# NILOIDE/A.I.gar

Measured on AMD Instinct MI355X. Metric: env-steps/sec at 4096 bots x 100k pellets; 1/2/4/8 MI355X scaling, higher is better.
Workload: dtype f64; 1 GPU; C3: 4096 bots, 100000 pellets, 1152 viruses, split p=0.0025, eject p=0.01, field 4800, obs 854 floats/bot; start: data/c3_t50.npz (tick 50, mean cell mass 17.45, max 51.3) + 30 untimed random-policy ticks to settle; policy=random, parallelism=single-gpu

## Files before the change

aigar_amd/csrc/aigar_dev.h:

```cpp
#pragma once
#include <stdint.h>

#include "../../include/aigar.h"

namespace aigar {

#ifdef AIGAR_FLOOR
#ifdef AIGAR_FLOOR_OPAQUE
#define FLOOR(k) \
  if ((((AIGAR_FLOOR) >> (k)) & 1) && d.A > 0) return
#else
#define FLOOR(k) \
  if (((AIGAR_FLOOR) >> (k)) & 1) return
#endif
#else
#define FLOOR(k)
#endif

struct ArenaCtl {
  int64_t seq_next;
  int64_t tick;
  int64_t tick_sp;
  uint64_t key0, key1, ctr_pellet, ctr_virus;
  int64_t seq_base_upd;
// ... 20 lines not shown
  double vmin_mass;
  uint64_t ev_order;
  uint32_t food_round;
  uint32_t scan_epoch[2];
  int scan_ticket[2];
  int src_n_stage;
  int n_kill;
  int pu_nconv;
  int pu_nsp, pu_spec;
  uint32_t dirty;
  int food_undone[3];
  uint32_t pl_epoch;
  int pl_ticket;
  int n_pel_glob, n_eaten_glob, n_out, n_out_pel, n_undone, n_undone_glob;
  int n_ho;
  int n_ho_live;
  int n_cmd;
  int64_t stat[8];
};

enum : uint32_t {
  ERR_PELLET_CAP = 1, ERR_BLOB_CAP = 2, ERR_VIRUS_CAP = 4, ERR_EVENT_CAP = 8, ERR_WORK_CAP = 16,
  ERR_OBS_CAP = 32, ERR_CAND_CAP = 64, ERR_SLOT = 128, ERR_PIX_CAP = 256, ERR_TILE_CAP = 512, ERR_TILE_LOOKUP = 1024,
  ERR_TILE_OBS = 2048,
  ERR_TILE_PASSES = 4096,
  ERR_PREDICT = 8192,
  ERR_TILE_HANDOFF = 16384
};
enum : uint32_t {
  WARN_NEW_VIRUS_EATS = 1, WARN_DEAD_VIRUS = 2, WARN_TILE_OBS = 4,
  WARN_Q_NONFINITE = 8,
  WARN_NOISE_NONFINITE = 16,
  WARN_NOISE_EXHAUSTED = 32,
  WARN_TRAIN_NONFINITE = 64
};
enum : uint32_t { DIRTY_VIRUS = 1, DIRTY_BLOB = 2 };

enum : uint32_t { PH_MERGE = 0, PH_VB = 1, PH_PV = 2, PH_PELLET = 3, PH_BLOB = 4, PH_PP = 5, PH_SPAWN = 6 };

struct TileRec {
  int32_t kind, idx;
  int64_t seq;
  double x, y;
};
enum : int32_t { TR_HDR = 0, TR_PELLET = 1, TR_BLOB = 2, TR_CELL = 3, TR_HIST = 4, TR_CMD = 5 };
constexpr int kHcapMax = 256;

struct alignas(32) PelRec {
  double x, y, m;
  int64_t seq;
};
constexpr int kPelStride = 4;
__device__ __forceinline__ void pel_store(PelRec *p, const PelRec &r) {
#ifdef AIGAR_PEL_WT
  __hip_atomic_store(&p->x, r.x, __ATOMIC_RELAXED, __HIP_MEMORY_SCOPE_AGENT);
  __hip_atomic_store(&p->y, r.y, __ATOMIC_RELAXED, __HIP_MEMORY_SCOPE_AGENT);
  __hip_atomic_store(&p->m, r.m, __ATOMIC_RELAXED, __HIP_MEMORY_SCOPE_AGENT);
  __hip_atomic_store(&p->seq, r.seq, __ATOMIC_RELAXED, __HIP_MEMORY_SCOPE_AGENT);
#else
  *p = r;
#endif
}

struct ScoreCtl {
  double *trace;
  int64_t cap;
};

struct Dev {
  int A, B, NP, size, cols, H;
  int tiled, tile_id, ntiles, tcap, bm_words;
  int tile_flags;
  int tile_nx, tile_ny;
  int tile_gate;
  int hcap, hrec, nh;
  int *t_holder;
  int *t_obsby;
  int *t_holive;
  uint8_t *t_hodefer;
  int *t_hoslot;
  int own_bx0, own_bx1, own_by0, own_by1;
  int loc_bx0, loc_bx1, loc_by0, loc_by1;
  TileRec *outbox;
  const TileRec *inbox;
  int *ticket;
  int *kill_list;
  double *spec_x, *spec_y, *spec_m;
  double pow_n032[17];
  int cshift;
  int cshift_c;
  int Pcap, Ecap, Vcap, Wcap, EVcap;
  int PR;
  int PS;
  int PD;
  int PH1;
  int virus_enabled;
  double max_pellets, max_viruses;
  int G, L;
  uint32_t obs_ch, obs_ex;
  int flags;
  int pp_par;
  ArenaCtl *ctl;
  int *p_alive, *p_respawn, *p_ncells, *p_split, *p_eject, *p_pend;
  double *p_cmdx, *p_cmdy;
  double *p_fx, *p_fy, *p_fs, *p_mass;
  int *p_split_lh;
  uint8_t *p_role;
  int *p_time;
  double *o_last_mass;
  uint8_t *p_list;
  int *p_newc, *p_newb, *p_seqoff, *p_bloboff;
  int *p_heavy;
  double *c_x, *c_y, *c_m, *c_r, *c_vx, *c_vy, *c_svx, *c_svy, *c_mt;
  int *c_svc;
  uint32_t *c_flags;
  int64_t *c_seq;
  uint8_t *c_active;
  double *sp_r, *sp_svx, *sp_svy;
  double *sb_x, *sb_y, *sb_svx, *sb_svy;
  uint8_t *sb_slot;
  PelRec *pel;
  int *pel_col;
  PelRec *pn;
  int *pn_col;
  uint8_t *pel_dead;
  int *pel_rank;
  int *pstart;
  int *pncnt;
  uint64_t *pel_owner;
  double *b_x, *b_y, *b_m, *b_r, *b_vx, *b_vy, *b_svx, *b_svy;
  int *b_svc;
  int64_t *b_seq, *b_ej;
  int *b_col;
  uint32_t *b_flags;
  uint64_t *b_owner;
  int *bstart, *bitems, *b_rank;
  uint64_t *bmap;
  double *v_x, *v_y, *v_m, *v_r, *v_vx, *v_vy, *v_svx, *v_svy;
  int *v_svc;
  int64_t *v_seq;
  uint32_t *v_flags;
  int *v_active;
  int *vcnt, *vstart, *vitems, *v_rank;
  int *ccnt, *cstart, *citems, *c_rank;
  int *cgcnt;
  unsigned long long *occ;
  int *occ_cnt;
  int occ_words;
  int *dead;
  int *work, *work2;
  int *f_list;
  uint8_t *f_cnt;
  uint8_t *f_done;
  int *resp_slot;
  int *resp_list;
  int64_t *ev;
  double *o_lastfov;
  double *o_self_lf, *o_self_slf, *o_en_lf, *o_en_slf;
  double *o_act_cur, *o_act_prev;
  unsigned long long *scan_state;
  unsigned long long *pl_state;
  int pl_tiles;
  int scan_tiles;
  int OBcap;
  unsigned long long *ob_used;
  uint32_t *ob_epoch;
  int64_t *ob_seq;
  double *ob_m, *ob_r;
  uint32_t *ob_mask;
  uint8_t *ob_own;
  int *ob_perm;
  uint64_t *ob_wmask;
  double *sc;
  ScoreCtl *sc_ctl;
};
enum { SC_N = 0, SC_SUM = 1, SC_MAX = 2, SC_DEAD = 3 };

struct ArenaSel {
  const int *al;
  const uint64_t *seeds;
  uint64_t seed;
  int first, n;
  __device__ __forceinline__ int arena(int i) const { return al ? al[i] : first + i; }
  __device__ __forceinline__ uint64_t seed_of(int i) const { return seeds ? seeds[i] : seed; }
  __device__ __forceinline__ int key_arena(int i) const { return al ? 0 : first + i; }
};

constexpr int FCAP = 32;

struct RandomPolicy {
  int on;
  double ps, pe;
  uint64_t salt;
};

}
```

aigar_amd/csrc/api.hip:

```cpp
#include <dlfcn.h>
#include <hip/hip_runtime.h>

#include <algorithm>
#include <cmath>
#include <cstdarg>
#include <cstdio>
#include <cstdlib>
#include <cstring>
#include <string>
#include <type_traits>
#include <vector>

#include "../../include/aigar.h"
#include "aigar_dev.h"
#include "aigar_sem.h"

namespace aigar {
void launch_tick(const Dev &d, hipStream_t s, int rounds, int64_t *scr_k, int *scr_v,
                 const RandomPolicy *rp = nullptr);
void launch_tick_pre(const Dev &d, hipStream_t s, int64_t *scr_k, int *scr_v, const RandomPolicy *rp);
void launch_tick_post(const Dev &d, hipStream_t s, int64_t *scr_k, int *scr_v);
void launch_tile_pass(const Dev &d, hipStream_t s, int rounds, int64_t *scr_k, int *scr_v, int first);
void launch_tile_policy(const Dev &d, hipStream_t s, int greedy_split, uint8_t *mask, int cap);
void launch_tile_cmd_apply(const Dev &d, hipStream_t s, int box_recs);
// ... 375 lines not shown
  if (cfg->obs_channels & AIGAR_OBS_ALL &&
      cfg->obs_channels & (AIGAR_OBS_SELF_LF | AIGAR_OBS_SELF_SLF | AIGAR_OBS_ENEMY_LF | AIGAR_OBS_ENEMY_SLF))
    return fail("aigar_create: ALL_PLAYER_GRID with last-frame grids is undefined in the reference");
  if ((cfg->flags & AIGAR_FLAG_SCORE) &&
      (std::max(1, cfg->tile_x) * std::max(1, cfg->tile_y) > 1 || (cfg->tile_flags & AIGAR_TILE_FORCE)))
    return fail("aigar_create: AIGAR_FLAG_SCORE (the mass history score) is not kept on a tiled handle");
  int ndev = 0;
  HIPCHK(hipGetDeviceCount(&ndev));
  if (cfg->device < 0 || cfg->device >= ndev) return fail("aigar_create: device %d not present (%d devices)", cfg->device, ndev);
  HIPCHK(hipSetDevice(cfg->device));
  aigar_handle *h = new aigar_handle();
  h->cfg = *cfg;
  if (getenv("AIGAR_NO_GRAPH")) h->use_graph = false;
  if (const char *u = getenv("AIGAR_RUN_UNROLL")) h->run_unroll = std::max(1, std::min(64, atoi(u)));
  if (getenv("AIGAR_TILE_GRAPH")) h->tile_graph = true;
  h->d.pp_par = getenv("AIGAR_PP_SERIAL") ? 0 : 1;
  if (const char *r = getenv("AIGAR_FOOD_ROUNDS")) h->rounds = std::max(1, std::min(16, atoi(r)));
  Dev &d = h->d;
  d.A = cfg->n_arenas;
  d.B = cfg->bots_per_arena;
  d.NP = d.A * d.B;
  d.size = cfg->field_size > 0 ? cfg->field_size : (int)(75 * std::sqrt((double)d.B));
  d.cols = (int)std::ceil(d.size / 20.0);
  d.H = d.cols * d.cols;
  d.virus_enabled = cfg->virus_enabled ? 1 : 0;
  d.max_pellets = cfg->max_pellets >= 0 ? cfg->max_pellets : (double)d.size * d.size * 0.015;
  d.max_viruses = cfg->max_viruses >= 0 ? cfg->max_viruses : (double)d.size * d.size * 0.00005;
  if (!d.virus_enabled) d.max_viruses = 0;
  auto r64 = [](int v) { return (v + 63) / 64 * 64; };
  d.Ecap = r64(cfg->blob_cap > 0 ? cfg->blob_cap : 4 * d.B + 256);
  d.Pcap = r64(cfg->pellet_cap > 0 ? cfg->pellet_cap : (int)std::ceil(d.max_pellets) + d.Ecap + 64);
  d.Vcap = r64(cfg->virus_cap > 0 ? cfg->virus_cap : 2 * (int)std::ceil(d.max_viruses) + 64);
  if (d.cols > 1024) {
    delete h;
    return fail("aigar_create: field size %d: more than 1024 bucket rows", d.size);
  }
  d.PR = r64((int)std::ceil(1.25 * d.Pcap / d.cols) + 64);
  d.PS = 2 * d.cols * d.PR;
  d.PD = d.PS + d.Pcap;
  d.PH1 = d.cols * (d.cols + 1) + 1;
  d.Wcap = std::max(kMaxCells * d.B, std::max(d.Ecap, 4096));
  d.EVcap = cfg->event_cap > 0 ? cfg->event_cap : 65536;
  d.G = G;
  d.L = obs_len_of(*cfg);
  d.obs_ch = cfg->obs_channels;
  d.obs_ex = cfg->obs_extras;
  d.flags = cfg->flags;
  d.occ_words = (d.H + 63) / 64;
  d.scan_tiles = (d.H + 2047) / 2048;
  d.pl_tiles = (d.B + 255) / 256;
  const int tx = std::max(1, cfg->tile_x), ty = std::max(1, cfg->tile_y);
  d.ntiles = tx * ty;
  d.tiled = d.ntiles > 1 || (cfg->tile_flags & AIGAR_TILE_FORCE);
  d.own_bx0 = d.own_by0 = d.loc_bx0 = d.loc_by0 = 0;
  d.own_bx1 = d.own_by1 = d.loc_bx1 = d.loc_by1 = d.cols;
  if (d.tiled) {
    auto bad = [&](const char *m) {
      delete h;
      return fail("aigar_create: %s", m);
    };
    if (d.A != 1) return bad("a tiled handle steps one arena (n_arenas must be 1)");
    if (cfg->tile_id < 0 || cfg->tile_id >= d.ntiles) return bad("tile_id out of range");
    if (tx > d.cols || ty > d.cols) return bad("more tiles than hash buckets along a side");
    const int ix = cfg->tile_id % tx, iy = cfg->tile_id / tx;
    const int halo = cfg->tile_halo > 0 ? cfg->tile_halo : 400;
    const int hb = std::max(7, (halo + kBucket - 1) / kBucket);
    if (d.ntiles > 64) return bad("at most 64 tiles");
    d.tile_id = cfg->tile_id;
    d.tile_flags = cfg->tile_flags;
    d.own_bx0 = ix * d.cols / tx;
    d.own_bx1 = (ix + 1) * d.cols / tx;
    d.own_by0 = iy * d.cols / ty;
    d.own_by1 = (iy + 1) * d.cols / ty;
    d.loc_bx0 = std::max(0, d.own_bx0 - hb);
    d.loc_bx1 = std::min(d.cols, d.own_bx1 + hb);
    d.loc_by0 = std::max(0, d.own_by0 - hb);
    d.loc_by1 = std::min(d.cols, d.own_by1 + hb);
  }
  d.tile_nx = tx;
  d.tile_ny = ty;
  d.tile_gate = 0;
  d.tcap = cfg->tile_cap > 0 ? cfg->tile_cap : 2048;
  d.bm_words = (int)(((size_t)kMaxCells * d.NP + 255) / 256 * 4);
  {
    const uint32_t ch = cfg->obs_channels;
    d.nh = ((ch & (AIGAR_OBS_SELF_LF | AIGAR_OBS_SELF_SLF)) ? 1 : 0) + ((ch & AIGAR_OBS_SELF_SLF) ? 1 : 0) +
           ((ch & (AIGAR_OBS_ENEMY_LF | AIGAR_OBS_ENEMY_SLF)) ? 1 : 0) + ((ch & AIGAR_OBS_ENEMY_SLF) ? 1 : 0);
    d.hrec = 1 + (d.nh * G * G + 3) / 4;
    d.hcap = std::min(kHcapMax, std::max(16, d.tcap / 64));
  }
  h->box_recs = 1 + d.tcap + std::max(d.bm_words / 4, d.hcap * d.hrec);
  for (int k = 0; k <= kMaxCells; k++) d.pow_n032[k] = aigar_math::pow_glibc((double)k, 0.32);
  d.cshift = 3;
  while ((((d.cols + (1 << d.cshift) - 1) >> d.cshift) * ((d.cols + (1 << d.cshift) - 1) >> d.cshift)) > 4096)
    d.cshift++;
  d.cshift_c = 0;
  while ((((d.cols + (1 << d.cshift_c) - 1) >> d.cshift_c) * ((d.cols + (1 << d.cshift_c) - 1) >> d.cshift_c)) > 4096)
    d.cshift_c++;
  if (hipStreamCreateWithFlags(&h->stream, hipStreamNonBlocking) != hipSuccess) {
    delete h;
    return fail("hipStreamCreate failed");
  }
  const size_t A = d.A, NP = d.NP, C = (size_t)kMaxCells * NP, H1 = (size_t)d.H + 1, GG = (size_t)G * G;
  bool ok = true;
#define AL(field, T, n)                     \
  do {                                      \
    d.field = dalloc<T>(h, (n));            \
    ok = ok && d.field != nullptr;          \
  } while (0)
#ifndef AIGAR_NO_ARENA
  for (int pass = 0; pass < 2; pass++) {
    h->arena_sizing = pass == 0;
    if (pass == 1) {
      h->arena_size = h->arena_used;
      h->arena_used = 0;
      void *base = nullptr;
      if (hipMalloc(&base, h->arena_size) != hipSuccess) {
        ok = false;
        break;
      }
      h->allocs.push_back(base);
      (void)hipMemset(base, 0, h->arena_size);
      h->arena = (char *)base;
    }
#endif
  AL(ctl, ArenaCtl, A);
  AL(p_alive, int, NP); AL(p_respawn, int, NP); AL(p_ncells, int, NP); AL(p_split, int, NP); AL(p_eject, int, NP);
  AL(p_pend, int, NP); AL(p_cmdx, double, NP); AL(p_cmdy, double, NP); AL(p_list, uint8_t, C);
  AL(p_newc, int, NP); AL(p_heavy, int, NP); AL(p_newb, int, NP); AL(p_seqoff, int, NP); AL(p_bloboff, int, NP);
  AL(c_x, double, C); AL(c_y, double, C); AL(c_m, double, C); AL(c_r, double, C); AL(c_vx, double, C);
  AL(c_vy, double, C); AL(c_svx, double, C); AL(c_svy, double, C); AL(c_mt, double, C); AL(c_svc, int, C);
  AL(c_flags, uint32_t, C); AL(c_seq, int64_t, C); AL(c_active, uint8_t, C);
  AL(sp_r, double, C); AL(sp_svx, double, C); AL(sp_svy, double, C);
  AL(sb_x, double, C); AL(sb_y, double, C); AL(sb_svx, double, C); AL(sb_svy, double, C); AL(sb_slot, uint8_t, C);
  const size_t P = A * d.Pcap, PSA = A * d.PS, PDA = A * d.PD, PHA = A * d.PH1;
  AL(pel, PelRec, PSA); AL(pel_col, int, PSA);
  AL(pn, PelRec, P); AL(pn_col, int, P);
  AL(pel_dead, uint8_t, PDA); AL(pel_rank, int, P); AL(pncnt, int, PHA); AL(pstart, int, PHA);
  AL(pel_owner, uint64_t, PDA);
  const size_t E = A * d.Ecap, V = A * d.Vcap;
  AL(b_x, double, E); AL(b_y, double, E); AL(b_m, double, E); AL(b_r, double, E); AL(b_vx, double, E);
  AL(b_vy, double, E); AL(b_svx, double, E); AL(b_svy, double, E); AL(b_svc, int, E); AL(b_seq, int64_t, E);
  AL(b_ej, int64_t, E); AL(b_flags, uint32_t, E); AL(b_owner, uint64_t, E); AL(b_col, int, E);
  AL(bstart, int, A * H1); AL(bitems, int, E); AL(b_rank, int, E); AL(bmap, uint64_t, A * 64);
  AL(v_x, double, V); AL(v_y, double, V); AL(v_m, double, V); AL(v_r, double, V); AL(v_vx, double, V);
  AL(v_vy, double, V); AL(v_svx, double, V); AL(v_svy, double, V); AL(v_svc, int, V); AL(v_seq, int64_t, V);
  AL(v_flags, uint32_t, V); AL(v_active, int, V);
  AL(vcnt, int, A * H1); AL(vstart, int, A * H1); AL(vitems, int, V); AL(v_rank, int, V);
  AL(ccnt, int, A * H1); AL(cstart, int, A * H1); AL(citems, int, C); AL(c_rank, int, C);
  AL(cgcnt, int, A * 2 * 4100);
  AL(occ, unsigned long long, A * d.occ_words); AL(occ_cnt, int, A * d.H);
  AL(dead, int, NP); AL(work, int, A * d.Wcap); AL(work2, int, A * d.Wcap);
  AL(f_list, int, C * FCAP); AL(f_cnt, uint8_t, C); AL(f_done, uint8_t, C);
  AL(resp_slot, int, NP); AL(resp_list, int, NP);
  AL(ev, int64_t, A * d.EVcap * 5);
  AL(o_lastfov, double, NP); AL(o_self_lf, double, NP * GG); AL(o_self_slf, double, NP * GG);
  AL(o_en_lf, double, NP * GG); AL(o_en_slf, double, NP * GG); AL(o_act_cur, double, NP * 4);
  AL(o_act_prev, double, NP * 4);
  d.OBcap = (int)std::min<size_t>(std::max<size_t>(1u << 20, 64 * NP), (size_t)1 << 24);
  AL(scan_state, unsigned long long, 2 * A * d.scan_tiles);
  AL(pl_state, unsigned long long, A * d.pl_tiles);
  AL(ticket, int, 16);
  AL(kill_list, int, P); AL(spec_x, double, A * 64); AL(spec_y, double, A * 64); AL(spec_m, double, A * 64); 
  AL(ob_used, unsigned long long, 1);
  AL(ob_epoch, uint32_t, 1);
  AL(p_split_lh, int, NP);
  AL(p_role, uint8_t, NP);
  AL(p_time, int, NP);
  AL(o_last_mass, double, NP);
  if (d.tiled) {
    AL(t_holder, int, NP);
    AL(t_obsby, int, NP);
    AL(t_holive, int, NP);
    AL(t_hodefer, uint8_t, NP);
    AL(t_hoslot, int, d.hcap);
    AL(outbox, TileRec, h->box_recs);
    TileRec *ib = nullptr;
    ib = dalloc<TileRec>(h, (size_t)h->box_recs * d.ntiles);
    ok = ok && ib != nullptr;
    d.inbox = ib;
  }
  AL(p_fx, double, NP); AL(p_fy, double, NP); AL(p_fs, double, NP); AL(p_mass, double, NP); AL(ob_seq, int64_t, d.OBcap); AL(ob_m, double, d.OBcap); AL(ob_r, double, d.OBcap);
  AL(ob_mask, uint32_t, d.OBcap); AL(ob_own, uint8_t, d.OBcap); AL(ob_perm, int, d.OBcap);
  d.ob_wmask = nullptr;
  if (G > 16) AL(ob_wmask, uint64_t, 4 * (size_t)d.OBcap);
  d.sc = nullptr;
  d.sc_ctl = nullptr;
  if (cfg->flags & AIGAR_FLAG_SCORE) {
    AL(sc, double, 4 * NP);
    AL(sc_ctl, ScoreCtl, 1);
  }
#undef AL
  h->scr_k = dalloc<int64_t>(h, A * d.Wcap);
  h->scr_v = dalloc<int>(h, A * d.Wcap);
  h->d_cmd = dalloc<double>(h, NP * 4);
  h->d_mask = dalloc<uint8_t>(h, NP);
  h->d_nnmask = dalloc<uint8_t>(h, NP);
  h->d_stats = dalloc<double>(h, NP * 5);
  h->d_obs = dalloc<double>(h, NP * (size_t)d.L);
  h->d_rlist = dalloc<int>(h, A);
  h->d_rseed = dalloc<uint64_t>(h, A);
  if (d.sc) {
    h->d_score = dalloc<double>(h, NP * 4);
    ok = ok && h->d_score;
  }
  ok = ok && h->scr_k && h->scr_v && h->d_cmd && h->d_stats && h->d_obs && h->d_mask && h->d_nnmask && h->d_rlist &&
       h->d_rseed;
#ifndef AIGAR_NO_ARENA
  }
  h->arena_sizing = false;
  h->arena = nullptr;
#endif
  if (ok) (void)hipMemset(h->d_nnmask, 1, NP);
  if (ok && !d.tiled) {
    ok = hipHostMalloc((void **)&h->h_reset, aigar_handle::kResetSlots * A * 2 * sizeof(uint64_t),
                       hipHostMallocDefault) == hipSuccess;
    for (hipEvent_t &e : h->ev_reset) ok = ok && hipEventCreateWithFlags(&e, hipEventDisableTiming) == hipSuccess;
  }
  (void)hipEventCreate(&h->ev0);
  (void)hipEventCreate(&h->ev1);
  if (!ok) {
    free_all(h);
    delete h;
    return fail("aigar_create: device allocation failed");
  }
  if (hipDeviceSynchronize() != hipSuccess) {
    free_all(h);
    delete h;
    return fail("aigar_create: device synchronize failed");
  }
  *out = h;
  return 0;
}

extern "C" int aigar_destroy(aigar_handle *h) {
  if (!h) return 0;
  (void)hipSetDevice(h->cfg.device);
  if (h->stream) (void)hipStreamSynchronize(h->stream);
  free_all(h);
  delete h;
  return 0;
}

static int check_device_errors(aigar_handle *h) {
  std::vector<ArenaCtl> ctl(h->d.A);
  HIPCHK(hipMemcpyAsync(ctl.data(), h->d.ctl, sizeof(ArenaCtl) * h->d.A, hipMemcpyDeviceToHost, h->stream));
  HIPCHK(hipStreamSynchronize(h->stream));
  for (int a = 0; a < h->d.A; a++)
    if (ctl[a].err)
      return fail("device error bits 0x%x in arena %d (1 pellet cap, 2 blob cap, 4 virus cap, 8 event cap, "
                  "16 worklist cap, 32 observation cap, 64 candidate cap, 128 slot, 256 pixel-frame object cap, "
                  "512 tile message cap, 1024 tile record lookup, 2048 tile view beyond the held pellets, "
                  "4096 tiled tick ended with undone cells, 8192 new-cell / blob counts not as predicted, "
                  "16384 more dead bots to hand off than hand-off slots)",
                  ctl[a].err, a);
  return 0;
}

static size_t pix_hist_bytes(const aigar_handle *h) {
  return (h->pix.flags & AIGAR_PIX_LAST) ? sizeof(uint32_t) * h->d.NP * (size_t)h->pix.side * h->pix.side : 0;
}
__global__ void __launch_bounds__(256) k_pix_hist_clear_arenas(uint32_t *hist, size_t row, ArenaSel sel) {
  uint32_t *p = hist + (size_t)sel.arena(blockIdx.y) * row;
  for (size_t i = blockIdx.x * (size_t)blockDim.x + threadIdx.x; i < row; i += (size_t)gridDim.x * blockDim.x) p[i] = 0;
}
__global__ void __launch_bounds__(256) k_pix_hist_clear_bots(uint32_t *hist, size_t LL, size_t n, const uint8_t *mask) {
  const size_t i = blockIdx.x * (size_t)blockDim.x + threadIdx.x;
  if (i < n && (!mask || mask[i / LL])) hist[i] = 0;
}

__global__ void k_fill_d(double *p, size_t n, double v) {
  size_t i = blockIdx.x * (size_t)blockDim.x + threadIdx.x;
  if (i < n) p[i] = v;
}

static void restart_side_buffers(aigar_handle *h, const ArenaSel &sel) {
  const Dev &d = h->d;
  if (h->d_pix_hist) {
    const size_t row = (size_t)d.B * h->pix.side * h->pix.side;
    const unsigned nb = (unsigned)std::min<size_t>((row + 255) / 256, 256);
    hipLaunchKernelGGL(k_pix_hist_clear_arenas, dim3(nb, sel.n), dim3(256), 0, h->stream, h->d_pix_hist, row, sel);
  }
  if (h->exp.cap) hipLaunchKernelGGL(k_exp_clear_arenas, dim3(sel.n), dim3(256), 0, h->stream, h->exp.has_old, d.B, sel);
  if (h->noi.n_act)
    hipLaunchKernelGGL(k_noise_clear_arenas, dim3(sel.n), dim3(256), 0, h->stream, h->noi.ou, d.B * h->noi.n_act, sel);
}
static int tiles_restart(aigar_handle *h) {
  const Dev &d = h->d;
  if (!d.tiled) return 0;
  HIPCHK(hipMemsetAsync(d.t_holder, 0xFF, sizeof(int) * d.NP, h->stream));
  HIPCHK(hipMemsetAsync(d.t_obsby, 0xFF, sizeof(int) * d.NP, h->stream));
  HIPCHK(hipMemsetAsync(d.t_hodefer, 0, d.NP, h->stream));
  return 0;
}

extern "C" int aigar_reset(aigar_handle *h, uint64_t seed) {
  if (!h) return fail("null handle");
  HIPCHK(hipSetDevice(h->cfg.device));
  const ArenaSel sel{nullptr, nullptr, seed, 0, h->d.A};
  restart_side_buffers(h, sel);
  if (tiles_restart(h)) return -1;
  launch_restart(h->d, h->stream, sel);
  HIPCHK(hipGetLastError());
  return check_device_errors(h);
}

// ... 3441 lines not shown
```

aigar_amd/csrc/tick.hip:

```cpp
#include <hip/hip_runtime.h>

#include "aigar_dev.h"
#include "aigar_sem.h"
#include "aigar_wave.h"

namespace aigar {

#define GTID ((int)(blockIdx.x * blockDim.x + threadIdx.x))
#define TILE_GATE(d)                                          \
  do {                                                        \
    if ((d).tile_gate && (d).ctl[0].n_undone_glob == 0) return; \
  } while (0)

#ifdef AIGAR_PHASE_TIMING
constexpr int kPtWaves = 8192;
__device__ unsigned int g_ptw[9][kPtWaves][8];
__device__ unsigned int g_ptid[9][kPtWaves][2];
__device__ __forceinline__ void pt_ids(unsigned *o) {
  unsigned a, b;
  asm volatile("s_getreg_b32 %0, hwreg(HW_REG_HW_ID)" : "=s"(a));
  asm volatile("s_getreg_b32 %0, hwreg(HW_REG_XCC_ID)" : "=s"(b));
  o[0] = a;
  o[1] = b;
}
#define PT_BEGIN(PT_K)                                                                              \
  const unsigned long long pt0_ = wall_clock64();                                                   \
  const int pt_w_ = (blockIdx.x + blockIdx.y * gridDim.x) * (blockDim.x >> 6) + (threadIdx.x >> 6); \
  if ((threadIdx.x & 63) == 0 && pt_w_ < kPtWaves) {                                                \
    g_ptw[PT_K][pt_w_][0] = (unsigned)pt0_;                                                         \
    pt_ids(g_ptid[PT_K][pt_w_]);                                                                    \
  }
#define PT_MARK(k, m)                                                                               \
  do {                                                                                              \
    asm volatile("s_waitcnt vmcnt(0) lgkmcnt(0)" ::: "memory");                                     \
    if ((threadIdx.x & 63) == 0 && pt_w_ < kPtWaves) g_ptw[k][pt_w_][m] = (unsigned)(wall_clock64() - pt0_); \
  } while (0)
#define PT_PARAMS , unsigned long long pt0_, int pt_w_
#define PT_MARKW(k, m)                                                                              \
  do {                                                                                              \
    asm volatile("s_waitcnt vmcnt(0) lgkmcnt(0)" ::: "memory");                                     \
    if ((int)(threadIdx.x & 63) == __ffsll((long long)__ballot(1)) - 1 && pt_w_ < kPtWaves)         \
      g_ptw[k][pt_w_][m] = (unsigned)(wall_clock64() - pt0_);                                       \
  } while (0)
#define PA_DECL                                   \
  unsigned long long pa_t_ = wall_clock64();      \
  unsigned pa_acc_[8] = {0, 0, 0, 0, 0, 0, 0, 0}, pa_cnt_[8] = {0, 0, 0, 0, 0, 0, 0, 0}
#define PA_T(k)                                                         \
  do {                                                                  \
    asm volatile("s_waitcnt vmcnt(0) lgkmcnt(0)" ::: "memory");         \
    const unsigned long long pa_n_ = wall_clock64();                    \
    pa_acc_[k] += (unsigned)(pa_n_ - pa_t_);                            \
    pa_t_ = pa_n_;                                                      \
  } while (0)
#define PA_C(k) (pa_cnt_[k]++)
#define PA_ADD(k, v) (pa_cnt_[k] += (v))
#define PA_STORE(a)                                                             \
  if ((threadIdx.x & 63) == 0 && (a) < kPtWaves)                                \
    for (int k_ = 0; k_ < 8; k_++) {                                            \
      g_ptw[6][a][k_] += pa_acc_[k_];                                           \
      g_ptw[7][a][k_] += pa_cnt_[k_];                                           \
    }
#define PA_STORE_GROUP(a)                                                       \
  if ((threadIdx.x & 63) == 0 && 1024 + (a) < kPtWaves)                         \
    for (int k_ = 0; k_ < 8; k_++) {                                            \
      atomicAdd(&g_ptw[6][1024 + (a)][k_], pa_acc_[k_]);                        \
      atomicAdd(&g_ptw[7][1024 + (a)][k_], pa_cnt_[k_]);                        \
    }
#define PT_ARGS , pt0_, pt_w_
#define PT_SUB(k)                                                                                 \
  do {                                                                                            \
    asm volatile("s_waitcnt vmcnt(0) lgkmcnt(0)" ::: "memory");                                   \
    if (threadIdx.x == 0 && 2048 + blockIdx.x < kPtWaves)                                         \
      g_ptw[6][2048 + blockIdx.x][k] = (unsigned)(wall_clock64() - pt0_);                         \
  } while (0)
#else
#define PT_SUB(k)
#define PT_BEGIN(k)
#define PT_MARK(k, m)
#define PT_MARKW(k, m)
#define PT_PARAMS
#define PT_ARGS
#define PA_DECL
#define PA_STORE_GROUP(a)
#define PA_T(k)
#define PA_C(k)
#define PA_ADD(k, v)
#define PA_STORE(a)
#endif

__device__ __forceinline__ void set_err(const Dev &d, int a, uint32_t bit) { atomicOr(&d.ctl[a].err, bit); }

constexpr int SG_CAP = 4096;
constexpr int CG_STRIDE = SG_CAP + 4;
template <int KIND>
__device__ __forceinline__ void grid_small_build(const Dev &d, int a, int *cnt, int *sh);

__device__ bool last_block(int *ticket, int nblocks, bool acquire = true) {
  __shared__ int s_last;
  asm volatile("s_waitcnt vmcnt(0)" ::: "memory");
  __syncthreads();
  if (threadIdx.x == 0) {
    __builtin_amdgcn_fence(__ATOMIC_RELEASE, "agent");
    asm volatile("s_waitcnt vmcnt(0)" ::: "memory");
    const int t = __hip_atomic_fetch_add(ticket, 1, __ATOMIC_RELAXED, __HIP_MEMORY_SCOPE_AGENT);
    s_last = t == nblocks - 1;
    if (t == nblocks - 1) {
      __hip_atomic_store(ticket, 0, __ATOMIC_RELAXED, __HIP_MEMORY_SCOPE_AGENT);
      if (acquire) {
        __builtin_amdgcn_fence(__ATOMIC_ACQUIRE, "agent");
        asm volatile("s_waitcnt vmcnt(0)" ::: "memory");
      }
    }
  }
  __syncthreads();
  return s_last;
}
__device__ void agent_acquire_block(bool need) {
  if (!need) return;
  if (threadIdx.x == 0) {
    __builtin_amdgcn_fence(__ATOMIC_ACQUIRE, "agent");
    asm volatile("s_waitcnt vmcnt(0)" ::: "memory");
  }
  __syncthreads();
}
__device__ __forceinline__ int agent_load(const int *p) {
  return __hip_atomic_load(p, __ATOMIC_RELAXED, __HIP_MEMORY_SCOPE_AGENT);
}
__device__ bool last_block_relaxed(int *ticket, int nblocks) {
  __shared__ int s_last;
  asm volatile("s_waitcnt vmcnt(0)" ::: "memory");
  __syncthreads();
  if (threadIdx.x == 0) {
    const int t = __hip_atomic_fetch_add(ticket, 1, __ATOMIC_RELAXED, __HIP_MEMORY_SCOPE_AGENT);
    s_last = t == nblocks - 1;
    if (t == nblocks - 1) __hip_atomic_store(ticket, 0, __ATOMIC_RELAXED, __HIP_MEMORY_SCOPE_AGENT);
  }
  __syncthreads();
  return s_last;
}
__device__ bool last_block_sharded(int *tk, int nblocks) {
  __shared__ int s_last;
  asm volatile("s_waitcnt vmcnt(0)" ::: "memory");
  __syncthreads();
  if (threadIdx.x == 0) {
    __builtin_amdgcn_fence(__ATOMIC_RELEASE, "agent");
    asm volatile("s_waitcnt vmcnt(0)" ::: "memory");
    const int sh = blockIdx.x & 7, members = (nblocks - sh + 7) / 8, shards = min(8, nblocks);
    int last = 0;
    if (__hip_atomic_fetch_add(&tk[sh], 1, __ATOMIC_RELAXED, __HIP_MEMORY_SCOPE_AGENT) == members - 1) {
      __hip_atomic_store(&tk[sh], 0, __ATOMIC_RELAXED, __HIP_MEMORY_SCOPE_AGENT);
      __builtin_amdgcn_fence(__ATOMIC_ACQ_REL, "agent");
      asm volatile("s_waitcnt vmcnt(0)" ::: "memory");
      if (__hip_atomic_fetch_add(&tk[8], 1, __ATOMIC_RELAXED, __HIP_MEMORY_SCOPE_AGENT) == shards - 1) {
        __hip_atomic_store(&tk[8], 0, __ATOMIC_RELAXED, __HIP_MEMORY_SCOPE_AGENT);
        __builtin_amdgcn_fence(__ATOMIC_ACQUIRE, "agent");
        asm volatile("s_waitcnt vmcnt(0)" ::: "memory");
        last = 1;
      }
    }
    s_last = last;
  }
  __syncthreads();
  return s_last;
}

__device__ __forceinline__ void tile_out(const Dev &d, int32_t kind, int32_t idx, int64_t seq, double x, double y) {
  const int i = atomicAdd(&d.ctl[0].n_out, 1);
  if (i >= d.tcap) {
    atomicOr(&d.ctl[0].err, (uint32_t)ERR_TILE_CAP);
    return;
  }
  if (kind == TR_PELLET) atomicAdd(&d.ctl[0].n_out_pel, 1);
  TileRec &r = d.outbox[1 + i];
  r.kind = kind;
  r.idx = idx;
  r.seq = seq;
  r.x = x;
  r.y = y;
}

__device__ void ev_push_at(const Dev &d, int a, int64_t tick, uint32_t phase, uint64_t order, int code, int64_t x,
                           int64_t y) {
  if (!(d.flags & 1)) return;
  if (d.tiled && d.tile_id != 0 && phase != PH_PELLET && phase != PH_BLOB) return;
  int i = atomicAdd(&d.ctl[a].n_ev, 1);
  if (i >= d.EVcap) {
    set_err(d, a, ERR_EVENT_CAP);
    return;
  }
  int64_t *e = d.ev + ((size_t)a * d.EVcap + i) * 5;
  e[0] = (tick << 8) | phase;
  e[1] = (int64_t)order;
  e[2] = code;
  e[3] = x;
  e[4] = y;
}
__device__ void ev_push(const Dev &d, int a, uint32_t phase, uint64_t order, int code, int64_t x, int64_t y) {
  ev_push_at(d, a, d.ctl[a].tick, phase, order, code, x, y);
}

template <class F>
__device__ __forceinline__ void grid_visit(const int *start, const int *items, int cols, Rect q, int E, F f,
                                           int shift = 0) {
  if (q.x1 < q.x0 || q.y1 < q.y0) return;
  const Span g = grid_span(q, E, cols, shift);
  for (int by = g.by0; by <= g.by1; by++) {
    int lo = start[by * g.stride + g.bx0], hi = start[by * g.stride + g.bx1 + 1];
    for (int t = lo; t < hi; t++) f(items ? items[t] : t);
  }
}
__device__ __forceinline__ int expand_for(double rmax) { return (int)ceil((rmax + 1.0) / kBucket) + 1; }

__device__ __forceinline__ void update_virus(const Dev &d, int gi) {
  int a = gi / d.Vcap, i = gi - a * d.Vcap;
  if (i >= d.ctl[a].n_vir || !(d.v_flags[gi] & F_ALIVE)) return;
  int svc = d.v_svc[gi];
  double svx = d.v_svx[gi], svy = d.v_svy[gi], x = d.v_x[gi], y = d.v_y[gi];
  update_momentum(svc, svx, svy);
  update_pos(x, y, d.v_vx[gi], d.v_vy[gi], svx, svy, svc, (double)d.size, (double)d.size);
  d.v_svc[gi] = svc;
  d.v_svx[gi] = svx;
  d.v_svy[gi] = svy;
  d.v_x[gi] = x;
  d.v_y[gi] = y;
  d.v_flags[gi] |= F_INHASH;
}

__device__ __forceinline__ bool update_blob(const Dev &d, int gi, double &x, double &y) {
  int a = gi / d.Ecap, i = gi - a * d.Ecap;
  if (i >= d.ctl[a].n_blob || !(d.b_flags[gi] & F_ALIVE)) return false;
  if (d.b_svc[gi] == 0) {
    int j = atomicAdd(&d.ctl[a].n_pnew, 1);
    if (j >= d.Pcap) {
      set_err(d, a, ERR_PELLET_CAP);
      return false;
    }
    size_t pj = (size_t)a * d.Pcap + j;
    d.pn[pj] = PelRec{d.b_x[gi], d.b_y[gi], d.b_m[gi], d.b_seq[gi]};
    d.pn_col[pj] = d.b_col[gi];
    d.b_flags[gi] = 0;
    atomicOr(&d.ctl[a].dirty, DIRTY_BLOB);
    return false;
  }
  int svc = d.b_svc[gi];
  double svx = d.b_svx[gi], svy = d.b_svy[gi];
  x = d.b_x[gi];
  y = d.b_y[gi];
  update_momentum(svc, svx, svy);
  update_pos(x, y, d.b_vx[gi], d.b_vy[gi], svx, svy, svc, (double)d.size, (double)d.size);
  d.b_svc[gi] = svc;
  d.b_svx[gi] = svx;
  d.b_svy[gi] = svy;
  d.b_x[gi] = x;
  d.b_y[gi] = y;
  return true;
}
__device__ __forceinline__ int blob_cell(const Dev &d, double x, double y) {
  const int s = d.cshift, cc = (d.cols + (1 << s) - 1) >> s;
  return (center_bucket_coord(y, d.cols) >> s) * cc + (center_bucket_coord(x, d.cols) >> s);
}
__device__ __forceinline__ int *cgrid_counts(const Dev &d, int a, int row);
__device__ __forceinline__ void blob_count(const Dev &d, int a, size_t g, double x, double y) {
  const int b = blob_cell(d, x, y);
  d.b_rank[g] = (b << 12) | atomicAdd(&cgrid_counts(d, a, 1)[b], 1);
}

__device__ __forceinline__ void predicted_counts(int heavy, int n0, bool split, bool eject, int &nsplit, int &nb) {
  const int c36 = heavy & 0xFF, c70 = (heavy >> 8) & 0xFF, c35 = (heavy >> 16) & 0xFF;
  nsplit = split ? min(c36, kMaxCells - n0) : 0;
  nb = eject ? 2 * min(nsplit, c70) + (c36 - nsplit) + c35 : 0;
}
struct CellIn {
  double m, r, svx, svy, mt, x, y;
  int svc;
};
__device__ __forceinline__ CellIn load_cell(const Dev &d, size_t ci) {
  return CellIn{d.c_m[ci], d.c_r[ci], d.c_svx[ci], d.c_svy[ci], d.c_mt[ci], d.c_x[ci], d.c_y[ci], d.c_svc[ci]};
}
__device__ __forceinline__ void update_cell(const Dev &d, size_t ci, const CellIn &in, double cmdx, double cmdy,
                                            bool split, int *heavy) {
  double m = in.m, r = in.r, svx = in.svx, svy = in.svy;
  const double mt = in.mt, x = in.x, y = in.y;
  int svc = in.svc;
  if (m >= 4) {
    m = m * kDecay;
    r = radius_of(m);
    d.c_m[ci] = m;
    d.c_r[ci] = r;
  }
  if (m >= 35)
    atomicAdd(heavy, (m > 36 ? 1 : 0) | (m >= 70 ? 1 << 8 : 0) | (m > 36 ? 0 : 1 << 16));
  update_momentum(svc, svx, svy);
  d.c_svc[ci] = svc;
  d.c_svx[ci] = svx;
  d.c_svy[ci] = svy;
  if (mt > 0) d.c_mt[ci] = mt - 1;
  double vx, vy, ca, sa;
  set_move_direction(x, y, m, r, cmdx, cmdy, vx, vy, ca, sa);
  d.c_vx[ci] = vx;
  d.c_vy[ci] = vy;
  if (split && m > 36) {
    const double W = (double)d.size, nr = radius_of(m / 2);
    const double xp = ca * nr * 4.5 + x, yp = sa * nr * 4.5 + y;
    double svx2, svy2;
    int svc2;
    add_momentum(x, y, xp, yp, W, W, r, svx2, svy2, svc2);
    d.sp_r[ci] = nr;
    d.sp_svx[ci] = svx2;
    d.sp_svy[ci] = svy2;
// ... 805 lines not shown
  }
  __syncthreads();
  PT_MARK(1, 5);
  const int64_t seq0 = s_seq0;
  const int blob0 = s_blob0;
  if (tile == ntiles - 1 && tid == 0) {
    const int tot = s_ps + s_ts, totb = s_pb + s_tb;
    c.seq_base_upd = seq0;
    c.seq_next = seq0 + tot;
    __hip_atomic_store(&c.n_blob_base, blob0, __ATOMIC_RELAXED, __HIP_MEMORY_SCOPE_AGENT);
    __hip_atomic_store(&c.n_blob_add, totb, __ATOMIC_RELAXED, __HIP_MEMORY_SCOPE_AGENT);
  }
  if (p < d.B && (fast || hslot >= 0 ? nb > 0 || nn > 0 : d.p_alive[gp] != 0)) {
    const int64_t s0 = seq0 + s_ps + ws[w] + (is - vs);
    const int boff = s_pb + wb[w] + (ib - vb);
    if (hslot >= 0) {
      const int n = s_hn[hslot];
      for (int k = n - nn; k < n; k++) d.c_seq[(size_t)s_hl[hslot][k] * NP + gp] = s0 + (k - (n - nn));
    } else if (fast) {
#pragma unroll
      for (int k = 0; k < kTailRegs; k++)
        if (k >= fn - nn && k < fn) d.c_seq[(size_t)flst[k] * NP + gp] = s0 + (k - (fn - nn));
    } else {
      const int n = d.p_ncells[gp];
      for (int k = 0; k < n; k++) {
        size_t ci = (size_t)d.p_list[k * NP + gp] * NP + gp;
        if (k >= n - nn) d.c_seq[ci] = s0 + (k - (n - nn));
        d.c_flags[ci] = (d.c_flags[ci] & ~F_NEW) | F_INHASH;
      }
    }
    for (int j = 0; j < nb; j++) {
      int bi = blob0 + boff + j;
      if (bi >= d.Ecap) break;
      size_t g = (size_t)a * d.Ecap + bi, si = (size_t)j * NP + gp;
      const double bm = kEjectMass * 0.8, bx = d.sb_x[si], by = d.sb_y[si];
      d.b_x[g] = bx;
      d.b_y[g] = by;
      d.b_m[g] = bm;
      d.b_r[g] = radius_of(bm);
      d.b_vx[g] = 0;
      d.b_vy[g] = 0;
      d.b_svx[g] = d.sb_svx[si];
      d.b_svy[g] = d.sb_svy[si];
      d.b_svc[g] = 15;
      d.b_seq[g] = s0 + nn + j;
      d.b_ej[g] = d.c_seq[(size_t)d.sb_slot[si] * NP + gp];
      d.b_col[g] = p;
      d.b_flags[g] = F_ALIVE;
      blob_count(d, a, g, bx, by);
    }
  }
  PT_MARK(1, 6);
  finish();
}


__device__ __forceinline__ int block_excl_1024(int x, int *wsum, int *total) {
  const int tid = threadIdx.x, lane = tid & 63, w = tid >> 6, nw = blockDim.x >> 6;
  int inc = x;
#pragma unroll
  for (int off = 1; off < 64; off <<= 1) {
    int y = __shfl_up(inc, off);
    if (lane >= off) inc += y;
  }
  if (lane == 63) wsum[w] = inc;
  __syncthreads();
  if (w == 0) {
    int v = lane < nw ? wsum[lane] : 0, vi = v;
#pragma unroll
    for (int off = 1; off < 16; off <<= 1) {
      int y = __shfl_up(vi, off);
      if (lane >= off) vi += y;
    }
    if (lane < nw) wsum[lane] = vi - v;
    if (lane == nw - 1) *total = vi;
  }
  __syncthreads();
  return inc - x + wsum[w];
}


template <int KIND>
__device__ __forceinline__ void grid_small_build(const Dev &d, int a, int *cnt, int *sh) {
  __shared__ double vmin_w[32];
  const int tid = threadIdx.x, T = blockDim.x, s = d.cshift;
  const int cc = (d.cols + (1 << s) - 1) >> s, Hc = cc * cc;
  ArenaCtl &c = d.ctl[a];
  const int per = KIND == 1 ? d.Ecap : d.Vcap;
  const int n = KIND == 1 ? c.n_blob : c.n_vir;
  __syncthreads();
  int *start = (KIND == 1 ? d.bstart : d.vstart) + (size_t)a * (d.H + 1);
  int *items = (KIND == 1 ? d.bitems : d.vitems) + (size_t)a * per;
  int *rank = (KIND == 1 ? d.b_rank : d.v_rank) + (size_t)a * per;
  for (int i = tid; i <= Hc; i += T) cnt[i] = 0;
  __syncthreads();
  double rloc = 0;
  for (int i = tid; i < n; i += T) {
    size_t g = (size_t)a * per + i;
    bool ok = (KIND == 1 ? d.b_flags[g] : d.v_flags[g]) & F_ALIVE;
    int rk = -1;
    if (ok) {
      double x = KIND == 1 ? d.b_x[g] : d.v_x[g], y = KIND == 1 ? d.b_y[g] : d.v_y[g];
      if (KIND == 2) rloc = fmax(rloc, d.v_r[g]);
      int b = (center_bucket_coord(y, d.cols) >> s) * cc + (center_bucket_coord(x, d.cols) >> s);
      rk = (b << 12) | atomicAdd(&cnt[b], 1);
    }
    rank[i] = rk;
  }
  if (KIND == 2) {
    double mn = __builtin_inf();
    for (int i = tid; i < n; i += T) {
      size_t g = (size_t)a * per + i;
      if (d.v_flags[g] & F_ALIVE) mn = fmin(mn, d.v_m[g]);
    }
#pragma unroll
    for (int off = 32; off > 0; off >>= 1) {
      mn = fmin(mn, __shfl_xor(mn, off));
      rloc = fmax(rloc, __shfl_xor(rloc, off));
    }
    if ((tid & 63) == 0) {
      vmin_w[tid >> 6] = mn;
      vmin_w[16 + (tid >> 6)] = rloc;
    }
  }
  __syncthreads();
  if (KIND == 2 && tid == 0) {
    double mn = vmin_w[0], rm = vmin_w[16];
    for (int k = 1; k < T >> 6; k++) {
      mn = fmin(mn, vmin_w[k]);
      rm = fmax(rm, vmin_w[16 + k]);
    }
    c.vmin_mass = mn;
    c.rmax_virus = rm;
  }
  block_scan_excl(cnt, cnt, Hc + 1, sh);
  for (int i = tid; i <= Hc; i += T) start[i] = cnt[i];
  for (int i = tid; i < n; i += T) {
    int rk = rank[i];
    if (rk < 0) continue;
    int b = rk >> 12, r = rk & 4095;
    if (r == 4095) set_err(d, a, ERR_SLOT);
    items[cnt[b] + r] = i;
  }
  __syncthreads();
}
__device__ __forceinline__ int cgrid_cols(const Dev &d) { return (d.cols + (1 << d.cshift_c) - 1) >> d.cshift_c; }
__device__ __forceinline__ int cgrid_bucket(const Dev &d, double x, double y) {
  const int sh = d.cshift_c;
  return (center_bucket_coord(y, d.cols) >> sh) * cgrid_cols(d) + (center_bucket_coord(x, d.cols) >> sh);
}
__device__ __forceinline__ int *cgrid_counts(const Dev &d, int a, int row) {
  return d.cgcnt + ((size_t)a * 2 + row) * CG_STRIDE;
}
__device__ __forceinline__ void cgrid_count_cell(const Dev &d, int a, size_t ci, double x, double y) {
  const int per = kMaxCells * d.B, slot = (int)(ci / d.NP), p = (int)(ci - (size_t)slot * d.NP) - a * d.B;
  const int b = cgrid_bucket(d, x, y);
  d.c_rank[(size_t)a * per + (size_t)slot * d.B + p] = (b << 17) | atomicAdd(&cgrid_counts(d, a, 0)[b], 1);
}
struct NoMid {
  __device__ void operator()() const {}
};
template <class Mid = NoMid>
__device__ void count_scan_256(int *cnt, int n, int *start, int *lds, uint16_t *bits, Mid mid = Mid()) {
  __shared__ int wsum[4];
  const int tid = threadIdx.x, lane = tid & 63, w = tid >> 6;
  const int4 *c4 = reinterpret_cast<const int4 *>(cnt);
  int v[16], sum = 0;
  int4 q4[4];
#pragma unroll
  for (int k = 0; k < 4; k++) {
    const int j = tid * 16 + 4 * k;
    q4[k] = j < n ? c4[j >> 2] : make_int4(0, 0, 0, 0);
  }
  mid();
#pragma unroll
  for (int k = 0; k < 4; k++) {
    const int j = tid * 16 + 4 * k;
    const int4 q = q4[k];
    v[4 * k] = j < n ? q.x : 0;
    v[4 * k + 1] = j + 1 < n ? q.y : 0;
    v[4 * k + 2] = j + 2 < n ? q.z : 0;
    v[4 * k + 3] = j + 3 < n ? q.w : 0;
  }
#pragma unroll
  for (int k = 0; k < 16; k++) sum += v[k];
  if (bits) {
    uint32_t bm = 0;
#pragma unroll
    for (int k = 0; k < 16; k++) bm |= (v[k] != 0 ? 1u : 0u) << k;
    bits[tid] = (uint16_t)bm;
  }
  int inc = sum;
#pragma unroll
  for (int off = 1; off < 64; off <<= 1) {
    int t = __shfl_up(inc, off);
    if (lane >= off) inc += t;
  }
  if (lane == 63) wsum[w] = inc;
  if constexpr (std::is_same<Mid, NoMid>::value) {
    __syncthreads();
  } else {
    __builtin_amdgcn_fence(__ATOMIC_RELEASE, "workgroup", "local");
    __builtin_amdgcn_s_barrier();
    __builtin_amdgcn_fence(__ATOMIC_ACQUIRE, "workgroup", "local");
  }
  int run = inc - sum;
  for (int k = 0; k < w; k++) run += wsum[k];
  const int total = wsum[0] + wsum[1] + wsum[2] + wsum[3];
#pragma unroll
  for (int k = 0; k < 16; k++) {
    const int j = tid * 16 + k;
    if (j < n) {
      start[j] = run;
      if (lds) lds[j] = run;
      cnt[j] = 0;
    }
    run += v[k];
  }
  if (tid == 0) {
    start[n] = total;
    if (lds) lds[n] = total;
  }
}
template <class Mid = NoMid>
__device__ __forceinline__ void cgrid_scan_block(const Dev &d, int a, Mid mid = Mid()) {
  const int cc = cgrid_cols(d);
  count_scan_256(cgrid_counts(d, a, 0), cc * cc, d.cstart + (size_t)a * (d.H + 1), nullptr, nullptr, mid);
}
__device__ __forceinline__ void cgrid_place_player(const Dev &d, int gp, int n) {
  const int NP = d.NP, a = gp / d.B, p = gp - a * d.B, per = kMaxCells * d.B;
  const int *start = d.cstart + (size_t)a * (d.H + 1);
  int *items = d.citems + (size_t)a * per;
  for (int k = 0; k < n; k++) {
    const int slot = d.p_list[k * NP + gp];
    const int br = d.c_rank[(size_t)a * per + (size_t)slot * d.B + p];
    items[start[br >> 17] + (br & 0x1FFFF)] = slot * NP + gp;
  }
}


__device__ __forceinline__ int prow_entry(const Dev &d, int bx, int by) { return by * (d.cols + 1) + bx; }
__device__ __forceinline__ void prow_count(const Dev &d, int a, int j) {
  const int gi = a * d.Pcap + j;
  ArenaCtl &c = d.ctl[a];
  if (j == 0) c.n_pel = 0;
  if (j >= c.n_pnew) return;
  const PelRec r = d.pn[gi];
  const int bx = center_bucket_coord(r.x, d.cols), by = center_bucket_coord(r.y, d.cols);
  d.pel_rank[gi] = tile_holds_bucket(d, bx, by) ? atomicAdd(&d.pncnt[(size_t)a * d.PH1 + prow_entry(d, bx, by)], 1) : -1;
}
__device__ __forceinline__ int block_scan4(int *v, int *wsum) {
  const int tid = threadIdx.x, lane = tid & 63, w = tid >> 6;
  int sum = v[0] + v[1] + v[2] + v[3], inc = sum;
#pragma unroll
  for (int off = 1; off < 64; off <<= 1) {
    const int y = __shfl_up(inc, off);
    if (lane >= off) inc += y;
  }
  if (lane == 63) wsum[w] = inc;
  __syncthreads();
  int before = 0, total = 0;
  for (int k = 0; k < 4; k++) {
    before += k < w ? wsum[k] : 0;
    total += wsum[k];
  }
  __syncthreads();
  int run = before + inc - sum;
  for (int k = 0; k < 4; k++) {
    const int x = v[k];
    v[k] = run;
    run += x;
  }
  return total;
}
__device__ __forceinline__ void prow_scan(const Dev &d, int r, int a) {
  __shared__ int wsum[4];
  const int tid = threadIdx.x, C = d.cols;
  ArenaCtl &c = d.ctl[a];
  int *cnt = d.pncnt + (size_t)a * d.PH1 + (size_t)r * (C + 1);
  int *st = d.pstart + (size_t)a * d.PH1 + (size_t)r * (C + 1);
  int v[4];
  for (int k = 0; k < 4; k++) {
    const int bx = tid * 4 + k;
    v[k] = bx < C ? cnt[bx] : 0;
  }
  const int total = block_scan4(v, wsum), base = r * d.PR;
  for (int k = 0; k < 4; k++) {
    const int bx = tid * 4 + k;
    if (bx < C) {
      st[bx] = base + min(v[k], d.PR);
      cnt[bx] = 0;
    }
  }
  if (tid == 0) {
    st[C] = base + min(total, d.PR);
    if (total > d.PR) set_err(d, a, ERR_PELLET_CAP);
    atomicAdd(&c.n_pel, min(total, d.PR));
    if (r == 0) {
      c.src_n_stage = c.n_pnew;
      c.n_pnew = 0;
      c.n_pel_eaten = 0;
    }
  }
}
__global__ void __launch_bounds__(256) k_prow_scan(Dev d, ArenaSel sel) {
  prow_scan(d, blockIdx.x, sel.arena(blockIdx.y));
}
__device__ __forceinline__ void prow_scatter(const Dev &d, int a, int j) {
  const int gi = a * d.Pcap + j;
  if (j >= d.ctl[a].src_n_stage) return;
  const int rk = d.pel_rank[gi];
  if (rk < 0) return;
  const PelRec r = d.pn[gi];
  const int bx = center_bucket_coord(r.x, d.cols), by = center_bucket_coord(r.y, d.cols);
  const int e = (int)((size_t)a * d.PH1) + prow_entry(d, bx, by);
  const int pos = d.pstart[e] + rk;
  if (pos >= d.pstart[e + 1]) return;
  const size_t o = (size_t)a * d.PS + pos;
  d.pel[o] = r;
  d.pel_col[o] = d.pn_col[gi];
}
__device__ __forceinline__ void merge_player(const Dev &d, int gp) {
  if (gp >= d.NP) return;
  const int NP = d.NP, a = gp / d.B;
  uint8_t l4[kTailRegs];
#pragma unroll
  for (int k = 0; k < kTailRegs; k++) l4[k] = d.p_list[k * NP + gp];
  const bool alive = d.p_alive[gp];
  const int n = d.p_ncells[gp];
  if (!alive) return;
  uint8_t cs[kMaxCells];
  int nm = 0;
  double mt4[kTailRegs];
#pragma unroll
  for (int k = 0; k < kTailRegs; k++) mt4[k] = k < n ? d.c_mt[(size_t)l4[k] * NP + gp] : 1.0;
#pragma unroll
  for (int k = 0; k < kTailRegs; k++)
    if (k < n && mt4[k] <= 0) cs[nm++] = l4[k];
  for (int k = kTailRegs; k < n; k++) {
    uint8_t s = d.p_list[k * NP + gp];
    if (d.c_mt[(size_t)s * NP + gp] <= 0) cs[nm++] = s;
  }
  if (nm <= 1) return;
  for (int i = 1; i < nm; i++) {
    uint8_t key = cs[i];
    double km = d.c_m[(size_t)key * NP + gp];
    int j = i - 1;
    while (j >= 0 && km > d.c_m[(size_t)cs[j] * NP + gp]) {
      cs[j + 1] = cs[j];
      j--;
    }
    cs[j + 1] = key;
  }
  uint32_t order = 0;
  for (int i = 0; i < nm; i++) {
    size_t c1 = (size_t)cs[i] * NP + gp;
    if (!(d.c_flags[c1] & F_ALIVE)) continue;
    for (int j = 0; j < nm; j++) {
      size_t c2 = (size_t)cs[j] * NP + gp;
      if (!(d.c_flags[c2] & F_ALIVE) || c2 == c1) continue;
      if (!overlap(d.c_x[c1], d.c_y[c1], d.c_m[c1], d.c_r[c1], d.c_x[c2], d.c_y[c2], d.c_m[c2], d.c_r[c2]))
        continue;
      bool first_big = d.c_m[c1] > d.c_m[c2];
      size_t bi = first_big ? c1 : c2, si = first_big ? c2 : c1;
      ev_push(d, a, PH_MERGE, ((uint64_t)(gp - a * d.B) << 20) | order++, 1, d.c_seq[bi], d.c_seq[si]);
      double m = grow_mass(d.c_m[bi], d.c_m[si]);
      d.c_m[bi] = m;
      d.c_r[bi] = radius_of(m);
      d.c_flags[si] = 0;
      uint8_t sslot = (uint8_t)(si / NP);
      int cur = d.p_ncells[gp], w = 0;
      for (int k = 0; k < cur; k++) {
        uint8_t s = d.p_list[k * NP + gp];
        if (s != sslot) d.p_list[(w++) * NP + gp] = s;
      }
      d.p_ncells[gp] = w;
      if (!(d.c_flags[c1] & F_ALIVE)) break;
    }
  }
}

__device__ double cgrid_count_player(const Dev &d, int gp) {
  const int NP = d.NP, a = gp / d.B;
  uint8_t l4[kTailRegs];
#pragma unroll
  for (int k = 0; k < kTailRegs; k++) l4[k] = d.p_list[k * NP + gp];
  const bool alive = d.p_alive[gp];
  const int n = d.p_ncells[gp];
  if (!alive) return 0.0;
  double rmax = 0;
  for (int k = 0; k < n; k++) {
    const size_t ci = (size_t)(k < kTailRegs ? l4[k] : d.p_list[k * NP + gp]) * NP + gp;
    cgrid_count_cell(d, a, ci, d.c_x[ci], d.c_y[ci]);
    rmax = fmax(rmax, d.c_r[ci]);
  }
  return rmax;
}

__device__ void isort_kv(int64_t *key, int *val, int n) {
  for (int i = 1; i < n; i++) {
    int64_t k = key[i];
    int v = val[i];
    int j = i - 1;
    while (j >= 0 && key[j] > k) {
      key[j + 1] = key[j];
      val[j + 1] = val[j];
      j--;
    }
    key[j + 1] = k;
    val[j + 1] = v;
  }
}

__device__ __forceinline__ void vb_active_blob(const Dev &d, int gb) {
  if (gb >= d.A * d.Ecap) return;
  const int a = gb / d.Ecap, j = gb - a * d.Ecap;
  const ArenaCtl &c = d.ctl[a];
  if (j >= c.n_blob || !(d.b_flags[gb] & F_ALIVE)) return;
  const double bx = d.b_x[gb], by = d.b_y[gb], bm = d.b_m[gb], br = d.b_r[gb];
  const Rect qb = footprint(bx, by, br, d.size);
  const int *st = d.vstart + (size_t)a * (d.H + 1);
  const int *it = d.vitems + (size_t)a * d.Vcap;
  const int nv = c.n_vir;
  grid_visit(st, it, d.cols, qb, expand_for(c.rmax_virus), [&](int i) {
    const size_t g = (size_t)a * d.Vcap + i;
    if (i >= nv || !(d.v_flags[g] & F_ALIVE)) return;
    const double vx = d.v_x[g], vy = d.v_y[g], vr = d.v_r[g];
    if (!rect_hit(footprint(vx, vy, vr, d.size), qb)) return;
    if (!overlap(vx, vy, d.v_m[g], vr, bx, by, bm, br)) return;
    if (atomicExch(&d.v_active[g], 1) != 0) return;
    const int w = atomicAdd(&d.ctl[a].n_pend, 1);
    if (w < d.Wcap) d.work[(size_t)a * d.Wcap + w] = i;
    else set_err(d, a, ERR_WORK_CAP);
  }, d.cshift);
}
__device__ void blob_grid_place(const Dev &d, int a, int *cnt) {
  const int tid = threadIdx.x, T = blockDim.x, s = d.cshift;
  const int cc = (d.cols + (1 << s) - 1) >> s;
  const int n = d.ctl[a].n_blob;
  int *items = d.bitems + (size_t)a * d.Ecap;
  const int *rank = d.b_rank + (size_t)a * d.Ecap;
  count_scan_256(cgrid_counts(d, a, 1), cc * cc, d.bstart + (size_t)a * (d.H + 1), cnt,
                 reinterpret_cast<uint16_t *>(d.bmap + (size_t)a * 64));
  __syncthreads();
  if (tid == 0) d.ctl[a].n_blob_live = cnt[cc * cc];
  for (int i = tid; i < n; i += T) {
    const int rk = rank[i];
    if (rk < 0) continue;
    const int b = rk >> 12, r = rk & 4095;
    if (r == 4095) set_err(d, a, ERR_SLOT);
    items[cnt[b] + r] = i;
  }
}
__device__ bool vb_serial_body(const Dev &d, int a, int64_t *scr_k, int *scr_v) {
  if ((threadIdx.x & 63) != 0) return false;
  ArenaCtl &c = d.ctl[a];
  int nw = min(agent_load(&c.n_pend), d.Wcap);
  c.n_pend = 0;
  c.stat[0] += nw;
  int *w = d.work + (size_t)a * d.Wcap;
  int64_t *ck = scr_k + (size_t)a * d.Wcap;
  int *cv = scr_v + (size_t)a * d.Wcap;
  if (nw == 0) return false;
  for (int k = 0; k < nw; k++) {
    ck[k] = w[k];
    d.v_active[(size_t)a * d.Vcap + w[k]] = 0;
  }
  isort_kv(ck, w, nw);
  const int *st = d.bstart + (size_t)a * (d.H + 1);
  const int *it = d.bitems + (size_t)a * d.Ecap;
  int wk = 0;
  uint64_t order = 0;
  const double thr = kVirusBase + 7 * kEjectMass * 0.8;
  for (int i = w[0]; i < c.n_vir; i++) {
    if (i < c.n_vir_start) {
      if (wk < nw && w[wk] == i) wk++;
      else continue;
    }
    size_t gv = (size_t)a * d.Vcap + i;
    double vx = d.v_x[gv], vy = d.v_y[gv];
    Rect q = footprint(vx, vy, d.v_r[gv], d.size);
    int nc = 0;
    grid_visit(st, it, d.cols, q, 1, [&](int j) {
      size_t g = (size_t)a * d.Ecap + j;
      if (!(d.b_flags[g] & F_ALIVE)) return;
      if (!rect_hit(footprint(d.b_x[g], d.b_y[g], d.b_r[g], d.size), q)) return;
      if (nc < d.Wcap) {
        ck[nc] = d.b_seq[g];
        cv[nc] = j;
        nc++;
      }
    }, d.cshift);
    isort_kv(ck, cv, nc);
    for (int t = 0; t < nc; t++) {
      size_t g = (size_t)a * d.Ecap + cv[t];
      if (!(d.b_flags[g] & F_ALIVE)) continue;
      if (!overlap(d.v_x[gv], d.v_y[gv], d.v_m[gv], d.v_r[gv], d.b_x[g], d.b_y[g], d.b_m[g], d.b_r[g])) continue;
      if (i >= c.n_vir_start) c.warn |= WARN_NEW_VIRUS_EATS;
      ev_push(d, a, PH_VB, order++, 2, d.v_seq[gv], d.b_seq[g]);
      double m = grow_mass(d.v_m[gv], d.b_m[g]);
      d.v_m[gv] = m;
      d.v_r[gv] = radius_of(m);
      c.rmax_virus = fmax(c.rmax_virus, d.v_r[gv]);
      d.b_flags[g] = 0;
      atomicOr(&d.ctl[a].dirty, DIRTY_BLOB);
      if (m >= thr) {
        if (c.n_vir >= d.Vcap) {
          c.err |= ERR_VIRUS_CAP;
          continue;
        }
        double ox = 2 * d.v_x[gv] - d.b_x[g], oy = 2 * d.v_y[gv] - d.b_y[g];
        size_t gn = (size_t)a * d.Vcap + c.n_vir;
        double x = d.v_x[gv], y = d.v_y[gv], nm = m / 2, nr = radius_of(nm);
        double ang = aigar_math::trig_atan2(oy - y, ox - x);
        double ca, sa;
        aigar_math::trig_sincos(ang, sa, ca);
        double xp = ca * nr * 4.5 + x, yp = sa * nr * 4.5 + y;
        double svx, svy;
        int svc;
        add_momentum(x, y, xp, yp, (double)d.size, (double)d.size, d.v_r[gv], svx, svy, svc);
        d.v_x[gn] = x;
        d.v_y[gn] = y;
        d.v_m[gn] = nm;
        d.v_r[gn] = nr;
        d.v_vx[gn] = 0;
        d.v_vy[gn] = 0;
        d.v_svx[gn] = svx;
        d.v_svy[gn] = svy;
        d.v_svc[gn] = svc;
        d.v_seq[gn] = c.seq_next++;
        d.v_flags[gn] = F_ALIVE;
        double pm = d.v_m[gv] / 2;
        d.v_m[gv] = pm;
        d.v_r[gv] = radius_of(pm);
        ev_push(d, a, PH_VB, order++, 3, d.v_seq[gv], d.v_seq[gn]);
        c.n_vir++;
      }
    }
  }
  return true;
}

__global__ void __launch_bounds__(256) k_merge_vb(Dev d, int64_t *scr_k, int *scr_v, int fold) {
  FLOOR(2);
  __shared__ int g_cnt[SG_CAP + 1];
  const int nbP = (d.NP + 255) / 256;
  if ((int)blockIdx.x >= nbP) {
    blob_grid_place(d, blockIdx.x - nbP, g_cnt);
  } else {
    const int gi = GTID;
    double rg = 0;
    if (gi < d.NP) {
      merge_player(d, gi);
      rg = cgrid_count_player(d, gi);
    }
    wave_atomic_max_pos(&d.ctl[min(gi, d.NP - 1) / d.B].rmax_cell, rg);
  }
  if (fold && last_block(d.ticket + 0, gridDim.x))
    for (int a = threadIdx.x >> 6; a < d.A; a += blockDim.x >> 6) vb_serial_body(d, a, scr_k, scr_v);
}

template <class Pred>
__device__ __forceinline__ bool wave_any_in_grid(const int *st, const int *items, int cols, Rect q, int E, Pred pred,
                                                 int shift = 0) {
  if (q.x1 < q.x0 || q.y1 < q.y0) return false;
  const Span g = grid_span(q, E, cols, shift);
  const int bx0 = g.bx0, bx1 = g.bx1, by0 = g.by0;
  const int lane = threadIdx.x & 63, nrows = g.by1 - by0 + 1;
  for (int r0 = 0; r0 < nrows; r0 += 64) {
    const int r = r0 + lane, nr = min(64, nrows - r0);
    int lo = 0, len = 0;
    if (r < nrows) {
      int b = (by0 + r) * g.stride;
      lo = st[b + bx0];
      len = st[b + bx1 + 1] - lo;
    }
    int inc = len;
#pragma unroll
    for (int off = 1; off < 64; off <<= 1) {
      int y = __shfl_up(inc, off);
      if (lane >= off) inc += y;
    }
    const int excl = inc - len, total = __shfl(inc, 63);
    for (int t0 = 0; t0 < total; t0 += 64) {
      const int t = t0 + lane;
      int row = 0;
      for (int k = 1; k < nr; k++) row = (__builtin_amdgcn_readlane(excl, k) <= t) ? k : row;
      const int idx = __shfl(lo, row) + (t - __shfl(excl, row));
      bool hit = t < total && pred(items ? items[idx] : idx);
      if (__ballot(hit)) return true;
    }
  }
  return false;
}

__device__ double pv_player(const Dev &d, int gp, bool count = true) {
  const int NP = d.NP, a = gp / d.B;
  const int *st = d.vstart + (size_t)a * (d.H + 1);
  const int *it = d.vitems + (size_t)a * d.Vcap;
  const int E = expand_for(d.ctl[a].rmax_virus);
  const double vmin = fmin(d.ctl[a].vmin_mass, kVirusBase);
  uint8_t l4[kTailRegs];
#pragma unroll
  for (int k = 0; k < kTailRegs; k++) l4[k] = d.p_list[k * NP + gp];
  const bool alive = d.p_alive[gp];
  const int n = d.p_ncells[gp];
  if (!alive) return 0.0;
  bool anyp = false;
  double rmax = 0;
  double x4[kTailRegs], y4[kTailRegs], m4[kTailRegs], r4[kTailRegs];
#pragma unroll
  for (int k = 0; k < kTailRegs; k++) {
    x4[k] = y4[k] = m4[k] = r4[k] = 0;
    if (k < n) {
      const size_t ci = (size_t)l4[k] * NP + gp;
      x4[k] = d.c_x[ci];
      y4[k] = d.c_y[ci];
      m4[k] = d.c_m[ci];
      r4[k] = d.c_r[ci];
    }
  }
  for (int k = 0; k < n; k++) {
    size_t ci;
    double x, y, m, r;
    if (k < kTailRegs) {
      uint8_t s = l4[0];
      x = x4[0], y = y4[0], m = m4[0], r = r4[0];
#pragma unroll
      for (int j = 1; j < kTailRegs; j++)
        if (k == j) s = l4[j], x = x4[j], y = y4[j], m = m4[j], r = r4[j];
      ci = (size_t)s * NP + gp;
    } else {
      ci = (size_t)d.p_list[k * NP + gp] * NP + gp;
      x = d.c_x[ci], y = d.c_y[ci], m = d.c_m[ci], r = d.c_r[ci];
    }
    rmax = fmax(rmax, r);
    bool any = false;
    if (m > 1.25 * vmin) {
      const Rect q = footprint(x, y, r, d.size);
      grid_visit(st, it, d.cols, q, E, [&](int j) {
        const size_t g = (size_t)a * d.Vcap + j;
        if (any || (d.v_flags[g] & (F_ALIVE | F_INHASH)) != (F_ALIVE | F_INHASH)) return;
        if (!rect_hit(footprint(d.v_x[g], d.v_y[g], d.v_r[g], d.size), q)) return;
        any = overlap(x, y, m, r, d.v_x[g], d.v_y[g], d.v_m[g], d.v_r[g]) && m > 1.25 * d.v_m[g];
      }, d.cshift);
    }
    d.c_active[ci] = any;
    anyp |= any;
  }
  if (anyp) {
    const int w = atomicAdd(&d.ctl[a].n_pend2, 1);
    if (w < d.Wcap) d.work2[(size_t)a * d.Wcap + w] = gp - a * d.B;
    else set_err(d, a, ERR_WORK_CAP);
  }
  if (count) {
#pragma unroll
    for (int k = 0; k < kTailRegs; k++)
      if (k < n) cgrid_count_cell(d, a, (size_t)l4[k] * NP + gp, x4[k], y4[k]);
    for (int k = kTailRegs; k < n; k++) {
      const size_t ci = (size_t)d.p_list[k * NP + gp] * NP + gp;
      cgrid_count_cell(d, a, ci, d.c_x[ci], d.c_y[ci]);
    }
  }
  return rmax;
}
__device__ void pv_redo(const Dev &d, int a) {
  const int lane = threadIdx.x & 63;
  asm volatile("s_waitcnt vmcnt(0)" ::: "memory");
  __builtin_amdgcn_fence(__ATOMIC_ACQUIRE, "agent");
  if (lane == 0) __hip_atomic_store(&d.ctl[a].n_pend2, 0, __ATOMIC_RELAXED, __HIP_MEMORY_SCOPE_AGENT);
  asm volatile("s_waitcnt vmcnt(0)" ::: "memory");
  for (int p = lane; p < d.B; p += 64) pv_player(d, a * d.B + p, false);
  asm volatile("s_waitcnt vmcnt(0)" ::: "memory");
  __builtin_amdgcn_fence(__ATOMIC_ACQUIRE, "agent");
}
__device__ void pv_serial_body(const Dev &d, int a, int64_t *scr_k, int *scr_v);
__global__ void __launch_bounds__(256) k_merge_pv(Dev d, int64_t *scr_k, int *scr_v) {
  FLOOR(2);
  __shared__ int g_cnt[SG_CAP + 1];
  const int nbP = (d.NP + 255) / 256, nbB = (d.A * d.Ecap + 255) / 256, b = blockIdx.x;
  if (b < nbP) {
    const int gi = GTID;
    double rg = 0;
    if (gi < d.NP) {
#ifndef AIGAR_DIAG_NO_MERGE
      merge_player(d, gi);
#endif
      rg = pv_player(d, gi);
    }
    wave_atomic_max_pos(&d.ctl[min(gi, d.NP - 1) / d.B].rmax_cell, rg);
  } else if (b < nbP + nbB) {
    vb_active_blob(d, (b - nbP) * 256 + threadIdx.x);
  } else {
    const int a = b - nbP - nbB;
    if (threadIdx.x == 0) d.ctl[a].n_vir_start = d.ctl[a].n_vir;
    blob_grid_place(d, a, g_cnt);
  }
  if (last_block(d.ticket + 0, gridDim.x, false)) {
    __shared__ int s_work;
    if (threadIdx.x == 0) {
      int w = 0;
      for (int a = 0; a < d.A; a++) w |= agent_load(&d.ctl[a].n_pend) | agent_load(&d.ctl[a].n_pend2);
      s_work = w;
    }
    __syncthreads();
    agent_acquire_block(s_work != 0);
    for (int a = threadIdx.x >> 6; a < d.A; a += blockDim.x >> 6) {
      const bool vb = vb_serial_body(d, a, scr_k, scr_v);
      if (__shfl(vb ? 1 : 0, 0)) pv_redo(d, a);
#ifndef AIGAR_DIAG_NO_PV_SERIAL
      pv_serial_body(d, a, scr_k, scr_v);
#endif
    }
  }
}
__device__ void pv_serial_body(const Dev &d, int a, int64_t *scr_k, int *scr_v) {
  const int lane = threadIdx.x & 63;
  const unsigned long long lt = (1ull << lane) - 1;
  ArenaCtl &c = d.ctl[a];
  int nw = min(agent_load(&c.n_pend2), d.Wcap);
  wave_fence();
  if (lane == 0) {
    c.n_pend2 = 0;
    c.stat[1] += nw;
  }
  if (nw == 0) return;
  const int NP = d.NP;
  int *w = d.work2 + (size_t)a * d.Wcap;
  int64_t *ck = scr_k + (size_t)a * d.Wcap;
  int *cv = scr_v + (size_t)a * d.Wcap;
  for (int k = 0; k < nw; k++) ck[k] = w[k];
  isort_kv(ck, w, nw);
  const int *st = d.vstart + (size_t)a * (d.H + 1);
  const int *it = d.vitems + (size_t)a * d.Vcap;
  const double W = (double)d.size;
  uint64_t order = 0;
  for (int wi = 0; wi < nw; wi++) {
    int gp = a * d.B + w[wi];
    if (!d.p_alive[gp]) continue;
    for (int i = 0; i < d.p_ncells[gp];) {
      size_t ci = (size_t)d.p_list[i * NP + gp] * NP + gp;
      i++;
      if (!d.c_active[ci] && !(d.c_flags[ci] & F_NEW)) continue;
      int E = expand_for(c.rmax_virus);
      Rect q = footprint(d.c_x[ci], d.c_y[ci], d.c_r[ci], d.size);
      int nc = 0;
      wave_grid_for(st, it, d.cols, q, E, [&](bool valid, int j) {
        bool keep = false;
        int64_t sq = 0;
        if (valid) {
          const size_t g = (size_t)a * d.Vcap + j;
          keep = (d.v_flags[g] & (F_ALIVE | F_INHASH)) == (F_ALIVE | F_INHASH) &&
                 rect_hit(footprint(d.v_x[g], d.v_y[g], d.v_r[g], d.size), q);
          if (keep) sq = d.v_seq[g];
        }
        const unsigned long long bal = __ballot(keep);
        const int slot = nc + __popcll(bal & lt);
        if (keep && slot < d.Wcap) {
          ck[slot] = sq;
          cv[slot] = j;
        }
        nc += __popcll(bal);
      }, d.cshift);
      nc = min(nc, d.Wcap);
      wave_fence();
      isort_kv(ck, cv, nc);
      for (int t = 0; t < nc; t++) {
        size_t g = (size_t)a * d.Vcap + cv[t];
        if (!(d.v_flags[g] & F_ALIVE)) continue;
        double cm = d.c_m[ci];
        if (!(overlap(d.c_x[ci], d.c_y[ci], cm, d.c_r[ci], d.v_x[g], d.v_y[g], d.v_m[g], d.v_r[g]) &&
              cm > 1.25 * d.v_m[g]))
          continue;
        if (lane == 0) ev_push(d, a, PH_PV, order, 4, d.c_seq[ci], d.v_seq[g]);
        order++;
        double m = grow_mass(cm, d.v_m[g] * kVirusEatFactor);
        d.c_m[ci] = m;
        d.c_r[ci] = radius_of(m);
        if (lane == 0) {
          atomic_max_pos(&c.rmax_cell, d.c_r[ci]);
          atomicOr(&d.ctl[a].dirty, DIRTY_VIRUS);
        }
        d.v_flags[g] = 0;
        int ncur = d.p_ncells[gp];
        int n_new = kMaxCells - ncur;
        if (lane == 0) ev_push(d, a, PH_PV, order, 5, d.c_seq[ci], n_new);
        order++;
        if (n_new == 0) continue;
        double dist = d.c_m[ci] * kExplosionProp;
        double mpc = dist / n_new;
        d.c_mt[ci] = merge_time_for(kMergeVirusFactor, d.c_m[ci]);
        double m2 = grow_mass(d.c_m[ci], -1 * mpc * n_new);
        d.c_m[ci] = m2;
        d.c_r[ci] = radius_of(m2);
        uint32_t used = 0;
        for (int k = 0; k < ncur; k++) used |= 1u << d.p_list[k * NP + gp];
        double px = d.c_x[ci], py = d.c_y[ci], pr = d.c_r[ci];
        for (int k = 0; k < n_new; k++) {
          int slot = __ffs(~used) - 1;
          used |= 1u << slot;
          size_t ni = (size_t)slot * NP + gp;
          int64_t seq = c.seq_next++;
          double nr = radius_of(mpc);
          uint64_t u[4];
          philox((uint64_t)seq, ST_ANGLE, 0, 0, c.key0, c.key1, u);
          int64_t deg = (int64_t)mulhi(u[0], 360);
          double ang = (double)deg * (kPi / 180.0);
          double ca, sa;
          aigar_math::trig_sincos(ang, sa, ca);
          double xp = ca * pr * 12 + px, yp = sa * pr * 12 + py;
          double vx, vy, svx, svy;
          int svc;
          set_move_direction(px, py, mpc, nr, xp, yp, vx, vy);
          add_momentum(px, py, xp, yp, W, W, pr, svx, svy, svc);
          d.c_x[ni] = px;
          d.c_y[ni] = py;
          d.c_m[ni] = mpc;
          d.c_r[ni] = nr;
          d.c_vx[ni] = vx;
          d.c_vy[ni] = vy;
          d.c_svx[ni] = svx;
          d.c_svy[ni] = svy;
          d.c_svc[ni] = svc;
          d.c_mt[ni] = merge_time_for(0.8, mpc);
          d.c_seq[ni] = seq;
          d.c_flags[ni] = F_ALIVE | F_INHASH | F_NEW;
          d.c_active[ni] = 0;
          if (lane == 0) cgrid_count_cell(d, a, ni, px, py);
          d.p_list[(ncur + k) * NP + gp] = (uint8_t)slot;
        }
        d.p_ncells[gp] = ncur + n_new;
      }
    }
    for (int k = 0; k < d.p_ncells[gp]; k++) d.c_flags[(size_t)d.p_list[k * NP + gp] * NP + gp] &= ~F_NEW;
  }
}

constexpr int kBlobBit = 1 << 30;
__device__ __forceinline__ void note_kill(const Dev &d, int a, int j) {
  const int k = atomicAdd(&d.ctl[a].n_kill, 1);
  if (k < d.Pcap) d.kill_list[(size_t)a * d.Pcap + k] = j;
  else set_err(d, a, ERR_PELLET_CAP);
}
struct Food {
  const Dev &d;
  int a;
  int n0, nst;
  int nblob;
  __device__ Food(const Dev &dd, int aa) : d(dd), a(aa), n0(dd.PS), nst(dd.ctl[aa].n_pnew), nblob(dd.ctl[aa].n_blob) {}
  __device__ static bool blob(int j) { return (j & kBlobBit) != 0; }
  __device__ size_t g(int j) const { return (size_t)a * d.PD + j; }
  __device__ size_t gp(int j) const { return (size_t)a * d.PS + j; }
  __device__ size_t gs(int j) const { return (size_t)a * d.Pcap + (j - n0); }
  __device__ size_t gb(int j) const { return (size_t)a * d.Ecap + (j & ~kBlobBit); }
  __device__ double x(int j) const { return blob(j) ? d.b_x[gb(j)] : (j < n0 ? d.pel[gp(j)].x : d.pn[gs(j)].x); }
  __device__ double y(int j) const { return blob(j) ? d.b_y[gb(j)] : (j < n0 ? d.pel[gp(j)].y : d.pn[gs(j)].y); }
  __device__ double m(int j) const { return blob(j) ? d.b_m[gb(j)] : (j < n0 ? d.pel[gp(j)].m : d.pn[gs(j)].m); }
  __device__ double r(int j) const { return blob(j) ? d.b_r[gb(j)] : pellet_radius(m(j)); }
  __device__ int64_t seq(int j) const {
    return blob(j) ? d.b_seq[gb(j)] : (j < n0 ? d.pel[gp(j)].seq : d.pn[gs(j)].seq);
  }
  __device__ void load(int j, double &x, double &y, double &m, int64_t &sq) const {
    if (blob(j)) {
      const size_t b = gb(j);
      x = d.b_x[b];
      y = d.b_y[b];
      m = d.b_m[b];
      sq = d.b_seq[b];
    } else {
      const PelRec r = j < n0 ? d.pel[gp(j)] : d.pn[gs(j)];
      x = r.x;
      y = r.y;
      m = r.m;
      sq = r.seq;
    }
  }
  __device__ double rad(int j, double m) const { return blob(j) ? d.b_r[gb(j)] : pellet_radius(m); }
  __device__ bool alive(int j) const { return blob(j) ? (d.b_flags[gb(j)] & F_ALIVE) != 0 : !d.pel_dead[g(j)]; }
  __device__ int64_t ej(int j) const { return blob(j) ? d.b_ej[gb(j)] : -2; }
  __device__ void mark_dead(int j) const {
    if (!blob(j)) {
      d.pel_dead[g(j)] = 1;
    } else {
      d.b_flags[gb(j)] = 0;
      atomicOr(&d.ctl[a].dirty, DIRTY_BLOB);
    }
  }
  __device__ void kill(int j) const {
    if (!blob(j)) {
      d.pel_dead[g(j)] = 1;
      if (j < n0) note_kill(d, a, j);
    } else {
      d.b_flags[gb(j)] = 0;
      atomicOr(&d.ctl[a].dirty, DIRTY_BLOB);
    }
  }
  __device__ uint64_t *owner(int j) const { return blob(j) ? d.b_owner + gb(j) : d.pel_owner + g(j); }
  __device__ bool any_blobs() const { return nblob > 0; }
  template <class Fn>
  __device__ void walk_pellets(Rect q, Fn f) const {
    wave_grid_for(d.pstart + (size_t)a * d.PH1, nullptr, d.cols, q, 1, f, 0, n0, nst, d.cols + 1);
  }
  template <class Fn>
  __device__ void walk_blobs(Rect q, Fn f) const {
    if (any_blobs())
      wave_grid_for(d.bstart + (size_t)a * (d.H + 1), d.bitems + (size_t)a * d.Ecap, d.cols, q, 1,
                    [&](bool valid, int j) { f(valid, valid ? (j | kBlobBit) : -1); }, d.cshift);
  }
  __device__ bool blobs_near(Rect q, const uint64_t *bm) const {
    if (!any_blobs() || q.x1 < q.x0 || q.y1 < q.y0) return false;
    const Span g = grid_span(q, 1, d.cols, d.cshift);
    const int w = g.bx1 - g.bx0 + 1, nb = w * (g.by1 - g.by0 + 1);
    bool any = false;
    for (int i = threadIdx.x & 63; i < nb; i += 64) {
      const int b = (g.by0 + i / w) * g.stride + g.bx0 + i % w;
      any |= (bm[b >> 6] >> (b & 63)) & 1;
    }
    return __ballot(any) != 0;
  }
  __device__ static int64_t order_key(int j, int64_t sq) { return sq | (blob(j) ? (1ll << 62) : 0); }
};
__device__ __forceinline__ uint64_t food_key(uint32_t round, uint32_t prio) {
  return ((uint64_t)round << 32) | (0xFFFFFFFFull - prio);
}
constexpr uint8_t kOverflow = 255;

__device__ __forceinline__ void wave_sync_lds() {
  __builtin_amdgcn_fence(__ATOMIC_RELEASE, "wavefront");
  __builtin_amdgcn_wave_barrier();
  __builtin_amdgcn_fence(__ATOMIC_ACQUIRE, "wavefront");
}
__device__ __forceinline__ double wave_sum(double v) {
#pragma unroll
  for (int off = 32; off > 0; off >>= 1) v += __shfl_xor(v, off);
  return v;
}

constexpr int PREP_CAND = 128;
constexpr int PREP_WAVES = 1;
__device__ __forceinline__ double tile_rall() { return sqrt(kMaxMass / kPi) * (1 + 1e-9); }
__global__ void __launch_bounds__(256, 4) k_food_prep(Dev d, int rounds, int resume) {
  FLOOR(4);
  TILE_GATE(d);
  __shared__ int64_t s_seq[4][PREP_CAND];
  __shared__ double s_x[4][PREP_CAND], s_y[4][PREP_CAND], s_m[4][PREP_CAND];
  __shared__ int s_idx[4][PREP_CAND];
  __shared__ uint8_t s_sel[4][PREP_CAND];
  __shared__ uint64_t s_bm[4][64];
  const bool head = !resume && (int)blockIdx.x < d.A;
  PT_BEGIN(0);
  const int w = threadIdx.x >> 6, lane = threadIdx.x & 63;
  const int wi = xcd_block(blockIdx.x, gridDim.x) * 4 + w, gp = wi / PREP_WAVES,
            h = wi - gp * PREP_WAVES;
  static_assert(PREP_WAVES == 1, "prep_multi assumes one wave per player");
  if (gp < d.NP && gp % d.B == 0 && h == 0 && lane == 0) d.ctl[gp / d.B].food_undone[1] = 0;
  if (gp >= d.NP && !head) return;
  const int gpl = min(gp, d.NP - 1);
  const int NP = d.NP, a = gpl / d.B;
  const int v_first = d.p_list[h * NP + gpl];
  const int v_slot = d.p_list[(lane < kMaxCells ? lane : 0) * NP + gpl];
  s_bm[w][lane] = d.bmap[(size_t)a * 64 + lane];
  const bool alive = d.p_alive[gpl];
  Food F(d, a);
  const uint32_t base = d.ctl[a].food_round;
  const int v_n = d.p_ncells[gpl];
  if (head) {
    double t0 = 0, t1 = 0, t2 = 0, t3 = 0;
    long long t4 = 0;
    cgrid_scan_block(d, blockIdx.x, [&] {
      if (gp < NP && alive && v_n > 0) {
        const size_t ci = (size_t)v_first * NP + gp;
        t0 = d.c_x[ci];
        t1 = d.c_y[ci];
        t2 = d.c_m[ci];
        t3 = d.c_r[ci];
        t4 = d.c_seq[ci];
      }
    });
    asm volatile("" ::"v"(t0), "v"(t1), "v"(t2), "v"(t3), "v"(t4));
    if (gp >= NP) return;
  }
  const int s_first = uni(v_first);
  const int n0 = uni(v_n);
  const int n = alive ? n0 : 0;
  PT_MARK(0, 1);
  auto prep_cell = [&](const int gpc, const int k, const size_t ci) {
    const int p = gpc - a * d.B;
    uint32_t prio = (uint32_t)p * kMaxCells + k;
    const size_t kc = (size_t)k * NP + gpc;
    if (resume && d.f_done[ci] == 1) return;
    double x = uni(d.c_x[ci]), y = uni(d.c_y[ci]), m = uni(d.c_m[ci]), r = uni(d.c_r[ci]);
    int64_t cseq = uni(d.c_seq[ci]);
    PT_MARK(0, 2);
    Rect q = uni(footprint(x, y, r, d.size));
    if (d.tiled && !tile_near_rect(d, rect_grow(footprint(x, y, fmax(r, tile_rall()), d.size), 1, d.cols), 2)) {
      if (lane == 0) {
        d.f_cnt[kc] = 0;
        d.f_done[ci] = 2;
      }
      return;
    }
    int cnt = 0;
    double lsum = 0;
    auto visit = [&](bool valid, int j) {
      bool keep = false;
      double fx = 0, fy = 0, fm = 0;
      int64_t fsq = 0;
      if (valid) {
        F.load(j, fx, fy, fm, fsq);
        keep = (!resume || F.alive(j)) && rect_hit(footprint(fx, fy, pellet_radius(fm), d.size), q);
      }
      unsigned long long bal = __ballot(keep);
      int slot = cnt + __popcll(bal & ((1ull << lane) - 1));
      if (keep) {
        lsum += fm;
        if (slot < PREP_CAND) {
          s_seq[w][slot] = Food::order_key(j, fsq);
          s_x[w][slot] = fx;
          s_y[w][slot] = fy;
          s_m[w][slot] = fm;
          s_idx[w][slot] = j;
        }
      }
      cnt += __popcll(bal);
    };
    F.walk_pellets(q, visit);
    PT_MARK(0, 3);
    const double Rp = fmax(r, radius_of(py_min(kMaxMass, (m + wave_sum(lsum)) * (1 + 1e-9))) * (1 + 1e-9));
    const Rect qb = uni(footprint(x, y, Rp, d.size));
    auto visit_b = [&](bool valid, int j) {
      bool keep = false;
      double fx = 0, fy = 0, fm = 0;
      int64_t fsq = 0;
      if (valid) {
        F.load(j, fx, fy, fm, fsq);
        keep = F.alive(j) && F.ej(j) != cseq && rect_hit(footprint(fx, fy, F.rad(j, fm), d.size), qb);
      }
      unsigned long long bal = __ballot(keep);
      int slot = cnt + __popcll(bal & ((1ull << lane) - 1));
      if (keep) {
        lsum += fm;
        if (slot < PREP_CAND) {
          s_seq[w][slot] = Food::order_key(j, fsq);
          s_x[w][slot] = fx;
          s_y[w][slot] = fy;
          s_m[w][slot] = fm;
          s_idx[w][slot] = j;
        }
      }
      cnt += __popcll(bal);
    };
    if (F.blobs_near(qb, s_bm[w])) F.walk_blobs(qb, visit_b);
    PT_MARK(0, 4);
    double sum = wave_sum(lsum);
    double M = uni(py_min(kMaxMass, (m + sum) * (1 + 1e-9)));
    double Rm = uni(fmax(r, radius_of(M)) * (1 + 1e-9));
    wave_sync_lds();
    if (d.tiled && (!(tile_holds_rect(d, rect_grow(q, 1, d.cols)) && tile_holds_rect(d, rect_grow(qb, 1, d.cols))) ||
                    ((d.tile_flags & AIGAR_TILE_OWNED_ONLY) && !tile_owns(d, x, y)))) {
      const uint64_t key = food_key(base + rounds + 2, prio);
      const Rect qm = footprint(x, y, fmax(r, tile_rall()), d.size);
      if (lane == 0) {
        d.f_cnt[kc] = kOverflow;
        d.f_done[ci] = 2;
      }
      F.walk_pellets(q, [&](bool valid, int j) {
        if (valid && F.alive(j) && rect_hit(footprint(F.x(j), F.y(j), F.r(j), d.size), q))
          atomicMax((unsigned long long *)F.owner(j), (unsigned long long)key);
      });
      F.walk_blobs(qm, [&](bool valid, int j) {
        if (valid && F.alive(j) && F.ej(j) != cseq && rect_hit(footprint(F.x(j), F.y(j), F.r(j), d.size), qm))
          atomicMax((unsigned long long *)F.owner(j), (unsigned long long)key);
      });
      return;
    }
    int nsel = 0;
    bool ovf = cnt > PREP_CAND;
    if (!ovf) {
      for (int i0 = 0; i0 < cnt; i0 += 64) {
        int i = i0 + lane;
        bool sel = false;
        if (i < cnt) {
          double fx = s_x[w][i], fy = s_y[w][i];
          sel = (M > 1.25 * s_m[w][i]) && ((x - fx) * (x - fx) + (y - fy) * (y - fy) < Rm * Rm);
          s_sel[w][i] = sel;
        }
        nsel += __popcll(__ballot(sel));
      }
      ovf = nsel > FCAP;
    }
    wave_sync_lds();
    PT_MARK(0, 5);
    if (ovf) {
      uint64_t key = food_key(base + rounds + 1, prio);
      if (lane == 0) {
        d.f_cnt[kc] = kOverflow;
        d.f_done[ci] = 0;
        int wi = atomicAdd(&d.ctl[a].n_pend, 1);
        if (wi < d.Wcap) {
          d.work[(size_t)a * d.Wcap + wi] = (int)ci;
          d.work2[(size_t)a * d.Wcap + wi] = (int)prio;
        } else {
          set_err(d, a, ERR_WORK_CAP);
        }
      }
      F.walk_pellets(q, [&](bool valid, int j) {
        if (valid && F.alive(j) && rect_hit(footprint(F.x(j), F.y(j), F.r(j), d.size), q))
          atomicMax((unsigned long long *)F.owner(j), (unsigned long long)key);
      });
      F.walk_blobs(qb, [&](bool valid, int j) {
        if (valid && F.alive(j) && rect_hit(footprint(F.x(j), F.y(j), F.r(j), d.size), qb))
          atomicMax((unsigned long long *)F.owner(j), (unsigned long long)key);
      });
      return;
    }
    int *lst = d.f_list + kc * FCAP;
    uint64_t key = food_key(base + 1, prio);
    for (int i0 = 0; i0 < cnt; i0 += 64) {
      int i = i0 + lane;
      if (i < cnt && s_sel[w][i]) {
        int64_t sq = s_seq[w][i];
        int rk = 0;
        for (int jj = 0; jj < cnt; jj++) rk += (s_sel[w][jj] && s_seq[w][jj] < sq);
        lst[rk] = s_idx[w][i];
        atomicMax((unsigned long long *)F.owner(s_idx[w][i]), (unsigned long long)key);
      }
    }
    if (lane == 0) {
      d.f_cnt[kc] = (uint8_t)nsel;
      d.f_done[ci] = (nsel == 0);
    }
    wave_sync_lds();
    PT_MARK(0, 6);
  };
  auto prep_multi = [&]() -> bool {
    const int n = uni(n0);
    const int g = lane >> 2, sub = lane & 3;
    const bool has = g < n;
    const int slot = __shfl(v_slot, g);
    const size_t ci = (size_t)(has ? slot : s_first) * NP + gp;
    const double x = d.c_x[ci], y = d.c_y[ci], m = d.c_m[ci], r = d.c_r[ci];
    PT_MARK(0, 2);
    const Rect q = footprint(x, y, r, d.size);
    const Span sp = grid_span(q, 1, d.cols, 0);
    const int ngrid = sp.by1 - sp.by0 + 1;
    const bool qok = has && q.x0 <= q.x1 && q.y0 <= q.y1;
    auto prefix = [&](int v, int &total) {
      int inc = v;
#pragma unroll
      for (int off = 1; off < 64; off <<= 1) {
        const int t = __shfl_up(inc, off);
        if (lane >= off) inc += t;
      }
      total = uni(__shfl(inc, 63));
      return inc - v;
    };
    int R;
    const int rbase = prefix(qok && sub == 0 ? ngrid + (F.nst > 0 ? 1 : 0) : 0, R);
    if (R > 64) return false;
    int c = 0;
    for (int k = 1; k < n; k++) c = (__builtin_amdgcn_readlane(rbase, 4 * k) <= lane) ? k : c;
    const int rr = lane - __shfl(rbase, 4 * c), c_by0 = __shfl(sp.by0, 4 * c), c_bx0 = __shfl(sp.bx0, 4 * c),
              c_bx1 = __shfl(sp.bx1, 4 * c), c_ng = __shfl(ngrid, 4 * c);
    int lo = 0, len = 0;
    if (lane < R) {
      if (rr < c_ng) {
        const int *st = d.pstart + (size_t)a * d.PH1;
        const int b = (c_by0 + rr) * (d.cols + 1);
        lo = st[b + c_bx0];
        len = st[b + c_bx1 + 1] - lo;
      } else {
        lo = F.n0;
        len = F.nst;
      }
    }
    int T;
    const int excl = prefix(len, T);
    int cnt = 0, pc = 0;
    for (int t0 = 0; t0 < T; t0 += 64) {
      const int t = t0 + lane;
      int row = 0;
      for (int k = 1; k < R; k++) row = (__builtin_amdgcn_readlane(excl, k) <= t) ? k : row;
      const int j = __shfl(lo, row) + (t - __shfl(excl, row)), cc = __shfl(c, row);
      const Rect qc{__shfl(q.x0, 4 * cc), __shfl(q.x1, 4 * cc), __shfl(q.y0, 4 * cc), __shfl(q.y1, 4 * cc)};
      bool keep = false;
      double fx = 0, fy = 0, fm = 0;
      int64_t fsq = 0;
      if (t < T) {
        F.load(j, fx, fy, fm, fsq);
        keep = rect_hit(footprint(fx, fy, pellet_radius(fm), d.size), qc);
      }
      const unsigned long long bal = __ballot(keep);
      const int at = cnt + __popcll(bal & ((1ull << lane) - 1));
      if (keep && at < PREP_CAND) {
        s_seq[w][at] = Food::order_key(j, fsq);
        s_x[w][at] = fx;
        s_y[w][at] = fy;
        s_m[w][at] = fm;
        s_idx[w][at] = j;
        s_sel[w][at] = (uint8_t)cc;
      }
      cnt += __popcll(bal);
      for (int k = 0; k < n; k++) {
        const int ck = __popcll(__ballot(keep && cc == k));
        pc += g == k ? ck : 0;
      }
    }
    PT_MARK(0, 3);
    if (cnt > PREP_CAND) return false;
    int all;
    const int ps = __shfl(prefix(sub == 0 ? pc : 0, all), lane & ~3);
    wave_sync_lds();
    double ls = 0;
    for (int i = sub; i < pc; i += 4) ls += s_m[w][ps + i];
    ls += __shfl_xor(ls, 1);
    ls += __shfl_xor(ls, 2);
    const double M = py_min(kMaxMass, (m + ls) * (1 + 1e-9));
    const double Rm = fmax(r, radius_of(M)) * (1 + 1e-9);
    bool near = false;
    const Rect qb = footprint(x, y, Rm, d.size);
    if (has && F.any_blobs() && qb.x0 <= qb.x1 && qb.y0 <= qb.y1) {
      const Span gb = grid_span(qb, 1, d.cols, d.cshift);
      const int bw = gb.bx1 - gb.bx0 + 1, nb = bw * (gb.by1 - gb.by0 + 1);
      for (int i = sub; i < nb; i += 4) {
        const int b = (gb.by0 + i / bw) * gb.stride + gb.bx0 + i % bw;
        near |= (s_bm[w][b >> 6] >> (b & 63)) & 1;
      }
    }
    if (__ballot(near)) return false;
    PT_MARK(0, 4);
    int nsel = 0;
    for (int i0 = 0; i0 < cnt; i0 += 64) {
      const int i = i0 + lane;
      const int cc = i < cnt ? s_sel[w][i] : 0;
      const double cx = __shfl(x, 4 * cc), cy = __shfl(y, 4 * cc), cM = __shfl(M, 4 * cc), cR = __shfl(Rm, 4 * cc);
      bool sel = false;
      if (i < cnt) {
        const double fx = s_x[w][i], fy = s_y[w][i];
        sel = (cM > 1.25 * s_m[w][i]) && ((cx - fx) * (cx - fx) + (cy - fy) * (cy - fy) < cR * cR);
      }
      for (int k = 0; k < n; k++) {
        const int ck = __popcll(__ballot(sel && cc == k));
        nsel += g == k ? ck : 0;
      }
      if (sel) s_sel[w][i] = (uint8_t)(cc | 0x80);
    }
    if (__ballot(has && nsel > FCAP)) return false;
    wave_sync_lds();
    PT_MARK(0, 5);
    const int p = gp - a * d.B;
    for (int i0 = 0; i0 < cnt; i0 += 64) {
      const int i = i0 + lane;
      const int tag = i < cnt ? s_sel[w][i] : 0, cc = tag & 0x7F;
      const int cps = __shfl(ps, 4 * cc), cpc = __shfl(pc, 4 * cc);
      if (tag & 0x80) {
        const int64_t sq = s_seq[w][i];
        int rk = 0;
        for (int jj = cps; jj < cps + cpc; jj++) rk += ((s_sel[w][jj] & 0x80) && s_seq[w][jj] < sq);
        const int j = s_idx[w][i];
        d.f_list[((size_t)cc * NP + gp) * FCAP + rk] = j;
        atomicMax((unsigned long long *)F.owner(j),
                  (unsigned long long)food_key(base + 1, (uint32_t)p * kMaxCells + cc));
      }
    }
    if (has && sub == 0) {
      d.f_cnt[(size_t)g * NP + gp] = (uint8_t)nsel;
      d.f_done[ci] = (nsel == 0);
    }
    PT_MARK(0, 6);
    return true;
  };
  if (n >= 2 && !resume && !d.tiled) {
    if (prep_multi()) return;
    wave_sync_lds();
  }
  for (int k = 0; k < n; k++) prep_cell(gp, k, (size_t)(k == 0 ? s_first : uni((int)d.p_list[k * NP + gp])) * NP + gp);
}
__device__ __forceinline__ void food_eat(const Dev &d, const Food &F, int a, int j, uint32_t prio, int t,
                                         int64_t cseq, int64_t fseq, double fm, double &m, double &r, int &eaten,
                                         bool own, double fx, double fy) {
  const bool bl = Food::blob(j);
  if (own) {
    ev_push(d, a, bl ? PH_BLOB : PH_PELLET, ((uint64_t)prio << 16) | (uint64_t)t, bl ? 7 : 6, cseq, fseq);
    if (d.tiled) {
      if (bl) tile_out(d, TR_BLOB, j & ~kBlobBit, fseq, 0.0, 0.0);
      else tile_out(d, TR_PELLET, 0, fseq, fx, fy);
    }
  }
  m = grow_mass(m, fm);
  r = radius_of(m);
  F.kill(j);
  eaten += bl ? 0 : 1;
}
struct FoodBatch {
  int j[kTailRegs];
  bool al[kTailRegs];
  double x[kTailRegs], y[kTailRegs], m[kTailRegs], r[kTailRegs];
  int64_t sq[kTailRegs];
  __device__ void load(const Dev &d, const Food &F, const int *jv, int n) {
#pragma unroll
    for (int k = 0; k < kTailRegs; k++) {
      j[k] = jv[k];
      al[k] = false;
      x[k] = y[k] = m[k] = r[k] = 0;
      sq[k] = 0;
      if (k < n) {
        al[k] = F.alive(j[k]);
        F.load(j[k], x[k], y[k], m[k], sq[k]);
        r[k] = Food::blob(j[k]) ? d.b_r[F.gb(j[k])] : 0.0;
      }
    }
  }
};
struct EaterIn {
  double x, y, m, r;
  int64_t seq;
};
__device__ double food_eat_loop(const Dev &d, const Food &F, int a, size_t ci, const EaterIn &cell, uint32_t prio,
                                const int *lst, int cnt, FoodBatch &fb) {
  const double x = cell.x, y = cell.y;
  double m = cell.m, r = cell.r;
  const int64_t cseq = cell.seq;
  const bool own = tile_owns(d, x, y);
  int eaten = 0;
  bool blobs = false, ate = false;
  Rect qb{};
  for (int t0 = 0; t0 < cnt; t0 += kTailRegs) {
    if (t0 > 0) {
      int jv[kTailRegs];
#pragma unroll
      for (int k = 0; k < kTailRegs; k++) jv[k] = t0 + k < cnt ? lst[t0 + k] : 0;
      fb.load(d, F, jv, cnt - t0);
    }
    int kp[kTailRegs], nkp = 0;
#pragma unroll
    for (int k = 0; k < kTailRegs; k++) {
      kp[k] = -1;
      const int t = t0 + k, j = fb.j[k];
      if (t >= cnt) continue;
      if (Food::blob(j) && !blobs) {
        blobs = true;
        qb = footprint(x, y, r, d.size);
      }
      if (!fb.al[k]) continue;
      const double fm = fb.m[k], fx = fb.x[k], fy = fb.y[k], fr = Food::blob(j) ? fb.r[k] : pellet_radius(fm);
      if (blobs && !rect_hit(footprint(fx, fy, fr, d.size), qb)) continue;
      if (!(overlap(x, y, m, r, fx, fy, fm, fr) && can_eat(m, fm))) continue;
      if (own) {
        const bool bl = Food::blob(j);
        ev_push(d, a, bl ? PH_BLOB : PH_PELLET, ((uint64_t)prio << 16) | (uint64_t)t, bl ? 7 : 6, cseq, fb.sq[k]);
        if (d.tiled) {
          if (bl) tile_out(d, TR_BLOB, j & ~kBlobBit, fb.sq[k], 0.0, 0.0);
          else tile_out(d, TR_PELLET, 0, fb.sq[k], fx, fy);
        }
      }
      m = grow_mass(m, fm);
      r = radius_of(m);
      F.mark_dead(j);
      if (!Food::blob(j)) {
        eaten++;
        if (j < F.n0) {
          kp[k] = j;
          nkp++;
        }
      }
      ate = true;
    }
    if (nkp) {
      int b = atomicAdd(&d.ctl[a].n_kill, nkp);
#pragma unroll
      for (int k = 0; k < kTailRegs; k++)
        if (kp[k] >= 0) {
          if (b < d.Pcap) d.kill_list[(size_t)a * d.Pcap + b] = kp[k];
          else set_err(d, a, ERR_PELLET_CAP);
          b++;
        }
    }
  }
  d.c_m[ci] = m;
  d.c_r[ci] = r;
  if (d.tiled && own && ate) tile_out(d, TR_CELL, (int32_t)ci, cseq, m, r);
  if (eaten) atomicAdd(&d.ctl[a].n_pel_eaten, eaten);
  return ate ? r : 0.0;
}
__device__ double food_commit_player(const Dev &d, int gp, int round, int last, int place PT_PARAMS) {
  const int NP = d.NP, a = gp / d.B, p = gp - a * d.B;
  ArenaCtl &c = d.ctl[a];
  const bool alive = d.p_alive[gp];
  const int n = d.p_ncells[gp];
  const int s_first = d.p_list[gp];
  const int cnt_first = d.f_cnt[gp];
  int l4_first[kTailRegs];
#pragma unroll
  for (int t = 0; t < kTailRegs; t++) l4_first[t] = d.f_list[(size_t)gp * FCAP + t];
  if (place && alive) cgrid_place_player(d, gp, n);
  if (round > 1 && c.food_undone[(round - 1) % 3] == 0) return 0;
  if (p == 0) c.food_undone[(round + 1) % 3] = 0;
  if (!alive) return 0;
  double rgrow = 0;
  Food F(d, a);
  for (int k = 0; k < n; k++) {
    const size_t kc = (size_t)k * NP + gp;
    const int *lst = d.f_list + kc * FCAP;
    int slot = s_first, cnt = cnt_first, l4[kTailRegs];
#pragma unroll
    for (int t = 0; t < kTailRegs; t++) l4[t] = l4_first[t];
    if (k > 0) {
      slot = d.p_list[kc];
      cnt = d.f_cnt[kc];
#pragma unroll
      for (int t = 0; t < kTailRegs; t++) l4[t] = lst[t];
    }
    PT_MARKW(4, 2);
    if (cnt == 0 || cnt == kOverflow) continue;
    const size_t ci = (size_t)slot * NP + gp;
    uint32_t prio = (uint32_t)p * kMaxCells + k;
    bool own = true;
    FoodBatch fb;
    EaterIn cell;
    bool done;
    {
      done = d.f_done[ci];
      cell.x = d.c_x[ci];
      cell.y = d.c_y[ci];
      cell.m = d.c_m[ci];
      cell.r = d.c_r[ci];
      cell.seq = d.c_seq[ci];
      uint64_t key = food_key(d.ctl[a].food_round + round, prio);
      uint64_t kw[kTailRegs];
#pragma unroll
      for (int t = 0; t < kTailRegs; t++) kw[t] = t < cnt ? *F.owner(l4[t]) : key;
      fb.load(d, F, l4, cnt);
#pragma unroll
      for (int t = 0; t < kTailRegs; t++) own &= kw[t] == key;
      if (done) continue;
      for (int t = kTailRegs; t < cnt && own; t++) own = (*F.owner(lst[t]) == key);
    }
    PT_MARKW(4, 3);
    if (own) {
      rgrow = fmax(rgrow, food_eat_loop(d, F, a, ci, cell, prio, lst, cnt, fb));
      d.f_done[ci] = 1;
      PT_MARKW(4, 4);
    } else if (!last) {
      uint64_t key = food_key(d.ctl[a].food_round + round + 1, prio);
      for (int t = 0; t < cnt; t++) atomicMax((unsigned long long *)F.owner(lst[t]), (unsigned long long)key);
      atomicAdd(&c.food_undone[round % 3], 1);
    } else {
      int w = atomicAdd(&d.ctl[a].n_pend, 1);
      if (w < d.Wcap) {
        d.work[(size_t)a * d.Wcap + w] = (int)ci;
        d.work2[(size_t)a * d.Wcap + w] = (int)prio;
      } else {
        set_err(d, a, ERR_WORK_CAP);
      }
    }
  }
  return rgrow;
}
__device__ void food_serial_body(const Dev &d, int a, int64_t *scr_k, int *scr_v, int rounds);
__global__ void __launch_bounds__(256) k_food_commit(Dev d, int round, int last, int64_t *scr_k, int *scr_v,
                                                     int rounds, int fold, int place) {
  FLOOR(5);
  TILE_GATE(d);
  const int ncommit = (d.NP + 255) / 256;
  PT_BEGIN(4);
  const int gp = GTID;
  const double rg = gp < d.NP ? food_commit_player(d, gp, round, last, place PT_ARGS) : 0.0;
  PT_MARK(4, round < 7 ? round : 7);
  wave_atomic_max_pos(&d.ctl[min(gp, d.NP - 1) / d.B].rmax_cell, rg);
  PT_MARK(4, 5);
  if (fold && last_block(d.ticket + 1, ncommit, false)) {
    __shared__ int s_work;
    if (threadIdx.x == 0) {
      int w = 0;
      for (int a = 0; a < d.A; a++) w |= agent_load(&d.ctl[a].n_pend);
      s_work = w;
    }
    __syncthreads();
    agent_acquire_block(s_work != 0);
    if (threadIdx.x < 64)
      for (int a = 0; a < d.A; a++) food_serial_body(d, a, scr_k, scr_v, rounds);
    PT_MARK(4, 6);
  }
}
constexpr int FS_CAP = 512;
__device__ void food_serial_body(const Dev &d, int a, int64_t *scr_k, int *scr_v, int rounds) {
  __shared__ int64_t s_key[FS_CAP];
  __shared__ int s_val[FS_CAP], s_srt[FS_CAP];
  __shared__ double s_x[FS_CAP], s_y[FS_CAP], s_m[FS_CAP], s_r[FS_CAP];
  const int lane = threadIdx.x & 63;
  ArenaCtl &c = d.ctl[a];
  const int nw = min(agent_load(&c.n_pend), d.Wcap);
  const uint32_t excl_round = c.food_round + rounds + 2;
  wave_fence();
  if (lane == 0) {
    c.n_pend = 0;
    c.stat[2] += nw;
    c.food_round += rounds + 2;
  }
  if (nw == 0) return;
  Food F(d, a);
  int *w = d.work + (size_t)a * d.Wcap;
  int *wp = d.work2 + (size_t)a * d.Wcap;
  if (nw <= FS_CAP) {
    for (int k = lane; k < nw; k += 64) {
      s_val[k] = w[k];
      s_key[k] = wp[k];
    }
    wave_fence();
    for (int k = lane; k < nw; k += 64) {
      int64_t key = s_key[k];
      int rk = 0;
      for (int y = 0; y < nw; y++) rk += s_key[y] < key;
      s_srt[rk] = k;
    }
    wave_fence();
    for (int k = lane; k < nw; k += 64) {
      w[k] = s_val[s_srt[k]];
      wp[k] = (int)s_key[s_srt[k]];
    }
  } else if (lane == 0) {
    int64_t *ck = scr_k + (size_t)a * d.Wcap;
    for (int k = 0; k < nw; k++) ck[k] = wp[k];
    isort_kv(ck, w, nw);
    for (int k = 0; k < nw; k++) wp[k] = (int)ck[k];
  }
  wave_fence();
  const unsigned long long lt = (1ull << lane) - 1;
  for (int wi = 0; wi < nw; wi++) {
    const size_t ci = (size_t)w[wi];
    const uint32_t prio = (uint32_t)wp[wi];
    const double x = d.c_x[ci], y = d.c_y[ci];
    double m = d.c_m[ci], r = d.c_r[ci];
    const int64_t cseq = d.c_seq[ci];
    const bool own = tile_owns(d, x, y);
    if (d.tiled) {
      const Rect q = footprint(x, y, r, d.size), qm = footprint(x, y, fmax(r, tile_rall()), d.size);
      bool taint = false;
      Rect box = q;
      auto check = [&](bool valid, int j) {
        bool hit = valid && F.alive(j) && F.ej(j) != cseq && rect_hit(footprint(F.x(j), F.y(j), F.r(j), d.size), box);
        if (hit) {
          const uint64_t w = *F.owner(j);
          hit = (uint32_t)(w >> 32) == excl_round && (0xFFFFFFFFu - (uint32_t)w) < prio;
        }
        if (__ballot(hit)) taint = true;
      };
      auto mark = [&](bool valid, int j) {
        if (valid && F.alive(j) && F.ej(j) != cseq && rect_hit(footprint(F.x(j), F.y(j), F.r(j), d.size), box))
          atomicMax((unsigned long long *)F.owner(j), (unsigned long long)food_key(excl_round, prio));
      };
      F.walk_pellets(q, check);
      box = qm;
      F.walk_blobs(qm, check);
      if (taint) {
        box = q;
        F.walk_pellets(q, mark);
        box = qm;
        F.walk_blobs(qm, mark);
        wave_fence();
        continue;
      }
    }
    int eaten = 0, t_base = 0;
    bool ate = false;
    for (int kind = 0; kind < 2; kind++) {
    const Rect q = footprint(x, y, r, d.size);
    int nc = 0;
    auto gather = [&](bool valid, int j) {
      double fx = 0, fy = 0, fm = 0, fr = 0;
      bool keep = valid && F.alive(j) && F.ej(j) != cseq;
      if (keep) {
        fx = F.x(j);
        fy = F.y(j);
        fm = F.m(j);
        fr = F.r(j);
        keep = rect_hit(footprint(fx, fy, fr, d.size), q);
      }
      unsigned long long bal = __ballot(keep);
      int slot = nc + __popcll(bal & lt);
      if (keep && slot < FS_CAP) {
        s_key[slot] = Food::order_key(j, F.seq(j));
        s_val[slot] = j;
        s_x[slot] = fx;
        s_y[slot] = fy;
        s_m[slot] = fm;
        s_r[slot] = fr;
      }
      nc += __popcll(bal);
    };
    if (kind == 0) F.walk_pellets(q, gather);
    else F.walk_blobs(q, gather);
    if (nc > FS_CAP) {
      set_err(d, a, ERR_CAND_CAP);
      nc = FS_CAP;
    }
    wave_fence();
    for (int k = lane; k < nc; k += 64) {
      int64_t key = s_key[k];
      int rk = 0;
      for (int y = 0; y < nc; y++) rk += s_key[y] < key;
      s_srt[rk] = k;
    }
    wave_fence();
    for (int t = 0; t < nc; t++) {
      const int k = s_srt[t];
      const double fm = s_m[k];
      if (!(overlap(x, y, m, r, s_x[k], s_y[k], fm, s_r[k]) && can_eat(m, fm))) continue;
      const int j = s_val[k];
      const int64_t fseq = s_key[k] & ~(1ll << 62);
      ate = true;
      if (lane == 0) {
        food_eat(d, F, a, j, prio, t_base + t, cseq, fseq, fm, m, r, eaten, own, s_x[k], s_y[k]);
      } else {
        m = grow_mass(m, fm);
        r = radius_of(m);
      }
    }
    t_base += nc;
    wave_fence();
    }
    if (lane == 0) {
      d.c_m[ci] = m;
      d.c_r[ci] = r;
      d.f_done[ci] = 1;
      if (d.tiled && own && ate) tile_out(d, TR_CELL, (int32_t)ci, cseq, m, r);
      if (eaten) atomicAdd(&d.ctl[a].n_pel_eaten, eaten);
      atomic_max_pos(&c.rmax_cell, r);
    }
    wave_fence();
  }
}
__global__ void __launch_bounds__(64) k_food_serial(Dev d, int64_t *scr_k, int *scr_v, int rounds) {
  TILE_GATE(d);
  food_serial_body(d, blockIdx.x, scr_k, scr_v, rounds);
}

__device__ __forceinline__ Rect cell_rect(const Dev &d, size_t ci) { return footprint(d.c_x[ci], d.c_y[ci], d.c_r[ci], d.size); }

__device__ __forceinline__ void occ_add(const Dev &d, int a, Rect q) {
  int *cnt = d.occ_cnt + (size_t)a * d.H;
  unsigned long long *occ = d.occ + (size_t)a * d.occ_words;
  const int w = q.x1 - q.x0 + 1, n = w * (q.y1 - q.y0 + 1);
  for (int t = threadIdx.x & 63; t < n; t += 64) {
    const int b = (q.y0 + t / w) * d.cols + q.x0 + t % w;
    atomicAdd(&cnt[b], 1);
    atomicOr(&occ[b >> 6], 1ull << (b & 63));
  }
}
__device__ __forceinline__ void occ_grow(const Dev &d, int a, Rect old, Rect q) {
  int *cnt = d.occ_cnt + (size_t)a * d.H;
  unsigned long long *occ = d.occ + (size_t)a * d.occ_words;
  const int w = q.x1 - q.x0 + 1, n = w * (q.y1 - q.y0 + 1);
  for (int t = threadIdx.x & 63; t < n; t += 64) {
    const int bx = q.x0 + t % w, by = q.y0 + t / w;
    if (bx >= old.x0 && bx <= old.x1 && by >= old.y0 && by <= old.y1) continue;
    const int b = by * d.cols + bx;
    if (atomicAdd(&cnt[b], 1) == 0) atomicOr(&occ[b >> 6], 1ull << (b & 63));
  }
}
__device__ __forceinline__ void occ_remove(const Dev &d, int a, Rect q) {
  int *cnt = d.occ_cnt + (size_t)a * d.H;
  unsigned long long *occ = d.occ + (size_t)a * d.occ_words;
  const int w = q.x1 - q.x0 + 1, n = w * (q.y1 - q.y0 + 1);
  for (int t = threadIdx.x & 63; t < n; t += 64) {
    const int b = (q.y0 + t / w) * d.cols + q.x0 + t % w;
    if (atomicSub(&cnt[b], 1) == 1) atomicAnd(&occ[b >> 6], ~(1ull << (b & 63)));
  }
}

constexpr int OCC_DW = 64;
#ifndef AIGAR_OCC_BATCH
#define AIGAR_OCC_BATCH 1
#endif
__device__ __forceinline__ void occ_mark(uint32_t *dirty, int b) {
  const int wd = b >> 6;
  atomicOr(&dirty[wd >> 5], 1u << (wd & 31));
}
__device__ __forceinline__ void occ_remove_def(const Dev &d, int a, Rect q, uint32_t *dirty) {
  int *cnt = d.occ_cnt + (size_t)a * d.H;
  const int w = q.x1 - q.x0 + 1, n = w * (q.y1 - q.y0 + 1);
  for (int t = threadIdx.x & 63; t < n; t += 64) {
    const int b = (q.y0 + t / w) * d.cols + q.x0 + t % w;
    (void)__hip_atomic_fetch_add(&cnt[b], -1, __ATOMIC_RELAXED, __HIP_MEMORY_SCOPE_AGENT);
    occ_mark(dirty, b);
  }
}
__device__ __forceinline__ void occ_grow_def(const Dev &d, int a, Rect old, Rect q, uint32_t *dirty) {
  int *cnt = d.occ_cnt + (size_t)a * d.H;
  const int w = q.x1 - q.x0 + 1, n = w * (q.y1 - q.y0 + 1);
  for (int t = threadIdx.x & 63; t < n; t += 64) {
    const int bx = q.x0 + t % w, by = q.y0 + t / w;
    if (bx >= old.x0 && bx <= old.x1 && by >= old.y0 && by <= old.y1) continue;
    const int b = by * d.cols + bx;
    (void)__hip_atomic_fetch_add(&cnt[b], 1, __ATOMIC_RELAXED, __HIP_MEMORY_SCOPE_AGENT);
    occ_mark(dirty, b);
  }
}
__device__ __forceinline__ void occ_rebuild_dirty(const Dev &d, int a, const uint32_t *dirty) {
  const int lane = threadIdx.x & 63, w = threadIdx.x >> 6, nw = blockDim.x >> 6;
  int *cnt = d.occ_cnt + (size_t)a * d.H;
  unsigned long long *occ = d.occ + (size_t)a * d.occ_words;
  static_assert(OCC_DW == 64, "one bitmap word per lane");
  const uint32_t mine = dirty[lane];
  unsigned long long nz = __ballot(mine != 0);
  int k = 0;
#if AIGAR_OCC_BATCH
  int q0 = -1, q1 = -1, q2 = -1, q3 = -1;
  auto word = [&](int wd, int c) {
    const unsigned long long bits = __ballot(c > 0);
    if (lane == 0) occ[wd] = bits;
  };
  auto flush = [&]() {
    auto ld = [&](int wd) {
      const int b = wd * 64 + lane;
      return wd >= 0 && b < d.H ? __hip_atomic_load(&cnt[b], __ATOMIC_RELAXED, __HIP_MEMORY_SCOPE_AGENT) : 0;
    };
    const int c0 = ld(q0), c1 = ld(q1), c2 = ld(q2), c3 = ld(q3);
    if (q0 >= 0) word(q0, c0);
    if (q1 >= 0) word(q1, c1);
    if (q2 >= 0) word(q2, c2);
    if (q3 >= 0) word(q3, c3);
    q0 = q1 = q2 = q3 = -1;
  };
#endif
  while (nz) {
    const int i = __ffsll((long long)nz) - 1;
    nz &= nz - 1;
    uint32_t m = (uint32_t)__builtin_amdgcn_readlane((int)mine, i);
    while (m) {
      const int wd = i * 32 + __ffs(m) - 1;
      m &= m - 1;
      if (k++ % nw != w) continue;
#if AIGAR_OCC_BATCH
      if (q0 < 0) q0 = wd;
      else if (q1 < 0) q1 = wd;
      else if (q2 < 0) q2 = wd;
      else {
        q3 = wd;
        flush();
      }
#else
      const int b = wd * 64 + lane;
      const int c = b < d.H ? __hip_atomic_load(&cnt[b], __ATOMIC_RELAXED, __HIP_MEMORY_SCOPE_AGENT) : 0;
      const unsigned long long bits = __ballot(c > 0);
      if (lane == 0) occ[wd] = bits;
#endif
    }
  }
#if AIGAR_OCC_BATCH
  if (q0 >= 0) flush();
#endif
}

__device__ __forceinline__ void pp_active_own(const Dev &d, int nblocks PT_PARAMS) {
  const int lane = threadIdx.x & 63;
  const int gp = xcd_block(blockIdx.x, nblocks) * 4 + (threadIdx.x >> 6);
  if (d.tiled && gp == 0 && lane == 0 && d.ctl[0].n_undone_glob != 0) atomicOr(&d.ctl[0].err, ERR_TILE_PASSES);
  if (gp >= d.NP) return;
  const int s_first = d.p_list[gp];
  const int v_slot = d.p_list[(lane < kMaxCells ? lane : 0) * d.NP + gp];
  if (!d.p_alive[gp]) return;
  const int NP = d.NP, a = gp / d.B;
  const int *st = d.cstart + (size_t)a * (d.H + 1);
  const int *it = d.citems + (size_t)a * kMaxCells * d.B;
  int E = expand_for(d.ctl[a].rmax_cell);
  int n = d.p_ncells[gp];
  bool anyp = false;
  PT_MARK(3, 1);
  auto pp_multi = [&]() -> bool {
    const int nu = uni(n);
    const bool has = lane < nu;
    const size_t ci = (size_t)(has ? v_slot : s_first) * NP + gp;
    const double x = d.c_x[ci], y = d.c_y[ci], m = d.c_m[ci], r = d.c_r[ci];
    PT_MARK(3, 2);
    const Rect q = footprint(x, y, r, d.size);
    const Span sp = grid_span(q, E, d.cols, d.cshift_c);
    const int nrow = has && q.x0 <= q.x1 && q.y0 <= q.y1 ? sp.by1 - sp.by0 + 1 : 0;
    auto prefix = [&](int v, int &total) {
      int inc = v;
#pragma unroll
      for (int off = 1; off < 64; off <<= 1) {
        const int t = __shfl_up(inc, off);
        if (lane >= off) inc += t;
      }
      total = uni(__shfl(inc, 63));
      return inc - v;
    };
// ... 1608 lines not shown
      if (i < hi) {
        if (live) {
          const int bx = bucket_of(i);
          const int pos = nb + s_nofs[bx] + (ex - s_lpre[bx]);
          if (pos < lim) {
            d.pel[S0 + pos] = d.pel[S0 + i];
            d.pel_col[S0 + pos] = d.pel_col[S0 + i];
          }
        } else {
          d.pel_dead[D0 + i] = 0;
        }
      }
    }
  }
  for (int k = tid; k < ns; k += PU_T) {
    const int j = s_sj[k], bx = s_sbx[k];
    int rk = 0;
    for (int q = 0; q < ns; q++) rk += s_sbx[q] == bx && s_sj[q] < j;
    const int pos = nb + s_nofs[bx] + s_live[bx] + rk;
    if (pos >= lim) continue;
    PelRec rec;
    int col = -1;
    if (k < PU_JREC) {
      rec = s_jrec[k];
      col = s_jcol[k];
    } else if (j >= nconv && spec) {
      const size_t o = (size_t)a * kSpawnAhead + (j - nconv);
      rec = PelRec{d.spec_x[o], d.spec_y[o], d.spec_m[o], c.seq_base_spawn + (j - nconv)};
    } else {
      rec = d.pn[Q0 + j];
      col = d.pn_col[Q0 + j];
    }
    d.pel[S0 + pos] = rec;
    d.pel_col[S0 + pos] = col;
  }
  if (over) {
    __syncthreads();
    for (int bx = tid; bx < C; bx += PU_T) s_lpre[bx] = 0;
    for (int c0 = 0; c0 < nst; c0 += PU_T) {
      const int j = c0 + tid;
      PelRec rec;
      int col = -1, bx = -1;
      if (j < nst) bx = staged(j, rec, col);
      s_sbx[tid] = (short)bx;
      __syncthreads();
      if (bx >= 0) {
        int rk = 0;
        for (int q = 0; q < tid; q++) rk += s_sbx[q] == bx;
        const int pos = nb + s_nofs[bx] + s_live[bx] + s_lpre[bx] + rk;
        if (pos < lim) {
          d.pel[S0 + pos] = rec;
          d.pel_col[S0 + pos] = col;
        }
      }
      __syncthreads();
      if (bx >= 0) atomicAdd(&s_lpre[bx], 1);
      __syncthreads();
    }
  }
  for (int bx = tid; bx < C; bx += PU_T) {
    const int st = nb + min(s_nofs[bx], d.PR);
    if (st != s_ost[bx]) e0[bx] = st;
  }
  if (tid == 0) {
    e0[C] = nb + min(total, d.PR);
    atomicAdd(&c.n_pel, min(total, d.PR) - (hi - lo));
  }
}
__global__ void __launch_bounds__(256) k_pel_update(Dev d, int nbF) {
  FLOOR(8);
  PT_BEGIN(8);
  const int nup = d.A * d.cols;
  if ((int)blockIdx.x >= nup + nbF) {
    spawn_virus(d, (blockIdx.x - nup - nbF) * 256 + threadIdx.x);
    PT_MARK(8, 5);
    return;
  }
  if ((int)blockIdx.x >= nup) {
    respawn_fov_thread(d, (blockIdx.x - nup) * 256 + threadIdx.x);
    PT_MARK(8, 4);
    return;
  }
  const int a = blockIdx.x / d.cols, r = blockIdx.x - a * d.cols;
  if (r == 0 && threadIdx.x == 0) d.ctl[a].tick += 1;
  __shared__ PelRowLds s_rows;
  pel_row_update(d, a, r, s_rows PT_ARGS);
  PT_MARK(8, 3);
}

__global__ void __launch_bounds__(256) k_pel_gather(Dev d, int a) {
  __shared__ int wsum[4];
  const int r = blockIdx.x, C = d.cols, tid = threadIdx.x;
  const int *pst = d.pstart + (size_t)a * d.PH1;
  int part = 0;
  for (int q = tid; q < r; q += blockDim.x) part += pst[(size_t)q * (C + 1) + C] - pst[(size_t)q * (C + 1)];
#pragma unroll
  for (int o = 32; o > 0; o >>= 1) part += __shfl_xor(part, o);
  if ((tid & 63) == 0) wsum[tid >> 6] = part;
  __syncthreads();
  const int off = wsum[0] + wsum[1] + wsum[2] + wsum[3];
  const int lo = pst[(size_t)r * (C + 1)], hi = pst[(size_t)r * (C + 1) + C];
  const size_t S0 = (size_t)a * d.PS, Q0 = (size_t)a * d.Pcap;
  for (int i = lo + tid; i < hi; i += blockDim.x) {
    const int o = off + (i - lo);
    if (o >= d.Pcap) break;
    d.pn[Q0 + o] = d.pel[S0 + i];
    d.pn_col[Q0 + o] = d.pel_col[S0 + i];
  }
}
void launch_pel_gather(const Dev &d, hipStream_t s, int a) {
  hipLaunchKernelGGL(k_pel_gather, dim3(d.cols), dim3(256), 0, s, d, a);
}

__device__ __forceinline__ void init_ctl(const Dev &d, ArenaCtl &c, uint64_t seed, int key_arena) {
  c.seq_next = d.B;
  c.tick = 0;
  c.key0 = seed;
  c.key1 = ((uint64_t)key_arena << 32) | 0x9E3779B9ull;
  c.ctr_pellet = c.ctr_virus = 0;
  c.n_pel = c.n_pnew = c.n_pel_eaten = 0;
  c.n_blob = c.n_blob_base = 0;
  c.n_vir = c.n_vir_start = 0;
  c.n_dead = 0;
  c.n_ev = 0;
  c.n_pend = c.n_pend2 = 0;
  c.n_kill = 0;
  c.pu_nconv = c.pu_nsp = c.pu_spec = 0;
  c.err = c.warn = 0;
  c.rmax_cell = radius_of(kStartMass);
  c.rmax_virus = radius_of(kVirusBase);
  c.food_round = 1;
  c.scan_epoch[0] = c.scan_epoch[1] = 0;
  c.pl_epoch = 0;
  c.dirty = 0;
  c.pl_ticket = 0;
  c.scan_ticket[0] = c.scan_ticket[1] = 0;
  c.n_pel_glob = c.n_eaten_glob = c.n_out = c.n_out_pel = c.n_undone = c.n_undone_glob = 0;
  c.n_ho = c.n_ho_live = 0;
  for (int k = 0; k < 8; k++) c.stat[k] = 0;
}


static inline int nblk(long n, int t) { return (int)((n + t - 1) / t); }

struct Scratch {
  int64_t *k;
  int *v;
};


static void launch_food(const Dev &d, hipStream_t s, int rounds, Scratch scr, int resume = 0, int fold = 0) {
  rounds = std::max(rounds, 1);
  const int g = nblk(d.NP, 256);
  hipLaunchKernelGGL(k_food_prep, dim3(std::max(nblk((long)d.NP * PREP_WAVES, 4), resume ? 0 : d.A)), dim3(256), 0, s, d,
                     rounds, resume);
  for (int r = 1; r <= rounds; r++) {
    hipLaunchKernelGGL(k_food_commit, dim3(g), dim3(256), 0, s, d, r, r == rounds ? 1 : 0, scr.k, scr.v, rounds,
                       fold && r == rounds ? 1 : 0, r == 1 && !resume ? 1 : 0);
  }
  if (!fold) hipLaunchKernelGGL(k_food_serial, dim3(d.A), dim3(64), 0, s, d, scr.k, scr.v, rounds);
}

void launch_tick_pre(const Dev &d, hipStream_t s, int64_t *scr_k, int *scr_v, const RandomPolicy *rp) {
  hipLaunchKernelGGL(k_players, dim3(d.pl_tiles + 1 + (d.Ecap + kPlT - 1) / kPlT, d.A), dim3(kPlT), 0, s, d, rp ? *rp : RandomPolicy{0, 0, 0, 0});
  if (d.virus_enabled)
    hipLaunchKernelGGL(k_merge_pv, dim3(nblk(d.NP, 256) + nblk((long)d.A * d.Ecap, 256) + d.A), dim3(256), 0, s, d,
                       scr_k, scr_v);
  else
    hipLaunchKernelGGL(k_merge_vb, dim3(nblk(d.NP, 256) + d.A), dim3(256), 0, s, d, scr_k, scr_v, 0);
}
static size_t pp_lds_bytes(const Dev &d) {
  return sizeof(uint32_t) * ((d.B + 31) / 32) * PPG_WAVES + (d.B <= PP_LOWN_MAX ? sizeof(int) * d.B : 0);
}
void launch_tick_post(const Dev &d, hipStream_t s, int64_t *scr_k, int *scr_v) {
  hipLaunchKernelGGL(k_pp_active, dim3(nblk(d.NP, 4)), dim3(256), 0, s, d, 0);
  hipLaunchKernelGGL(k_spawn_plan, dim3(d.A), dim3(1024), pp_lds_bytes(d), s, d, scr_k, scr_v, 1, 1);
  const int nbF = nblk(d.NP, 256);
  const int nbV = d.virus_enabled ? nblk((long)d.A * d.Vcap, 256) : 0;
  hipLaunchKernelGGL(k_pel_update, dim3(d.A * d.cols + nbF + nbV), dim3(256), 0, s, d, nbF);
}
void launch_score_sample(const Dev &d, hipStream_t s);
void launch_tick(const Dev &d, hipStream_t s, int rounds, int64_t *scr_k, int *scr_v, const RandomPolicy *rp) {
  if (d.sc) launch_score_sample(d, s);
  launch_tick_pre(d, s, scr_k, scr_v, rp);
  if (d.tiled) {
    launch_food(d, s, rounds, Scratch{scr_k, scr_v}, 0, 1);
    launch_tick_post(d, s, scr_k, scr_v);
    return;
  }
  launch_food(d, s, rounds, Scratch{scr_k, scr_v}, 0, 1);
  hipLaunchKernelGGL(k_pp_active, dim3(nblk(d.NP, 4) + d.A + nblk(d.NP, 256)), dim3(256), 0, s, d, 1);
  hipLaunchKernelGGL(k_spawn_plan, dim3(d.A + d.A * d.cols), dim3(1024), std::max(pp_lds_bytes(d), sizeof(PelRowLds)),
                     s, d, scr_k, scr_v, 1, 2);
}

__global__ void k_tile_pass_begin(Dev d) {
  ArenaCtl &c = d.ctl[0];
  c.n_out = c.n_out_pel = c.n_undone = 0;
  c.n_ho = c.n_ho_live = 0;
  TileRec &hd = d.outbox[0];
  hd.kind = TR_HDR;
  hd.idx = 0;
  hd.seq = 0;
  hd.x = hd.y = 0.0;
}
__device__ void tile_header(const Dev &d);
__global__ void __launch_bounds__(256) k_tile_collect(Dev d, int with_bitmap) {
  TILE_GATE(d);
  const int gp = GTID;
  if (gp < d.NP && d.p_alive[gp]) {
    unsigned long long *bm = (unsigned long long *)(d.outbox + 1 + d.tcap);
    const int NP = d.NP, n = d.p_ncells[gp];
    int und = 0;
    for (int k = 0; k < n; k++) {
      const size_t ci = (size_t)d.p_list[k * NP + gp] * NP + gp;
      if (!tile_owns(d, d.c_x[ci], d.c_y[ci])) continue;
      if (d.f_done[ci] != 1) und++;
      else if (with_bitmap) atomicOr(&bm[ci >> 6], 1ull << (ci & 63));
    }
    if (und) atomicAdd(&d.ctl[0].n_undone, und);
  }
  if (last_block(d.ticket + 3, gridDim.x)) {
    if (!with_bitmap) tile_plan_live(d);
    if (threadIdx.x == 0) tile_header(d);
  }
}
__device__ void tile_header(const Dev &d) {
  const ArenaCtl &c = d.ctl[0];
  TileRec &h = d.outbox[0];
  h.kind = TR_HDR;
  h.idx = min(c.n_out, d.tcap);
  h.seq = c.n_undone;
  h.x = (double)c.n_out_pel;
  h.y = (double)min(c.n_ho, d.hcap);
}
void launch_tile_pass(const Dev &d0, hipStream_t s, int rounds, int64_t *scr_k, int *scr_v, int first) {
  Dev d = d0;
  d.tile_gate = first ? 0 : 1;
  if (!first) hipLaunchKernelGGL(k_tile_pass_begin, dim3(1), dim3(1), 0, s, d);
  launch_food(d, s, rounds, Scratch{scr_k, scr_v}, first ? 0 : 1, 1);
  if (!first) (void)hipMemsetAsync(d.outbox + 1 + d.tcap, 0, 8 * (size_t)d.bm_words, s);
  hipLaunchKernelGGL(k_tile_collect, dim3(nblk(d.NP, 256)), dim3(256), 0, s, d, first ? 0 : 1);
}
__global__ void __launch_bounds__(256) k_tile_apply(Dev d, int box_recs, int first) {
  const int T = d.ntiles, k = blockIdx.x, tid = threadIdx.x;
  ArenaCtl &c = d.ctl[0];
  const TileRec *box = d.inbox + (size_t)k * box_recs;
  if (k == d.tile_id) {
    if (tid == 0) {
      int kills = 0, und = 0;
      for (int t = 0; t < T; t++) {
        const TileRec &h = d.inbox[(size_t)t * box_recs];
        kills += (int)h.x;
        und += (int)h.seq;
      }
      c.n_eaten_glob += kills;
      c.n_undone_glob = und;
      if (first) c.n_ho = c.n_ho_live = 0;
    }
    return;
  }
  const int nrec = min(box[0].idx, d.tcap);
  for (int i = tid; i < nrec; i += blockDim.x) {
    const TileRec r = box[1 + i];
    if (r.kind == TR_PELLET) {
      const int bx = center_bucket_coord(r.x, d.cols), by = center_bucket_coord(r.y, d.cols);
      if (!tile_holds_bucket(d, bx, by)) continue;
      const Food F(d, 0);
      const int e = by * (d.cols + 1) + bx, lo = d.pstart[e], hi = d.pstart[e + 1];
      bool found = false;
      for (int t = lo; t < hi && !found; t++)
        if (d.pel[F.gp(t)].seq == r.seq) {
          uint8_t *pd = d.pel_dead + F.g(t);
          unsigned *w = (unsigned *)((uintptr_t)pd & ~(uintptr_t)3);
          const unsigned sh = (unsigned)((uintptr_t)pd & 3) * 8;
          if (!((atomicOr(w, 1u << sh) >> sh) & 0xFFu)) note_kill(d, 0, t);
          found = true;
        }
      for (int j = F.n0; j < F.n0 + F.nst && !found; j++)
        if (d.pn[F.gs(j)].seq == r.seq) {
          d.pel_dead[F.g(j)] = 1;
          found = true;
        }
      if (!found) set_err(d, 0, ERR_TILE_LOOKUP);
    } else if (r.kind == TR_BLOB) {
      if (d.b_seq[r.idx] != r.seq) {
        set_err(d, 0, ERR_TILE_LOOKUP);
        continue;
      }
      d.b_flags[r.idx] = 0;
      atomicOr(&c.dirty, DIRTY_BLOB);
    } else if (r.kind == TR_CELL) {
      if (d.c_seq[r.idx] != r.seq) {
        set_err(d, 0, ERR_TILE_LOOKUP);
        continue;
      }
      d.c_m[r.idx] = r.x;
      d.c_r[r.idx] = r.y;
      d.f_done[r.idx] = 1;
      atomic_max_pos(&c.rmax_cell, r.y);
    }
  }
  if (first) {
    const int GG = d.G * d.G, per = d.nh * GG, slot_e = 1 + per, ns = min((int)box[0].y, d.hcap);
    for (int e = tid; e < ns * slot_e; e += blockDim.x) {
      const int sl = e / slot_e, j = e - sl * slot_e;
      const TileRec *slot = box + 1 + d.tcap + (size_t)sl * d.hrec;
      const int gp = slot->idx;
      if (slot->kind != TR_HIST || gp < 0 || gp >= d.NP) {
        set_err(d, 0, ERR_TILE_LOOKUP);
        continue;
// ... 202 lines not shown
```

Measured before the change: 50.95 million env-steps/s.

## Fold cell-grid scan into merge kernels and food commit rounds into prep

Moves the per-arena cell-grid prefix scan out of the food-prep head blocks and into the last block of the merge kernels, where one wave per arena scans the counts held in LDS planes. Cell placement into citems now happens inside food prep, using a rank index keyed by player and cell index. When folding is enabled and the run is not tiled, food prep records contested cells in a global list and its last block runs the commit rounds and the serial fallback itself, so the separate commit and serial kernel launches are skipped. This cuts launch count and grid-wide passes, but puts more serial work into a single last block and relies on relaxed atomics and agent-scope loads for correctness.

Result: slower. 43.97 million env-steps/s (-13.7%).

```diff
diff --git a/aigar_amd/csrc/aigar_dev.h b/aigar_amd/csrc/aigar_dev.h
--- a/aigar_amd/csrc/aigar_dev.h
+++ b/aigar_amd/csrc/aigar_dev.h
@@ -196,6 +196,8 @@
   int *f_list;
   uint8_t *f_cnt;
   uint8_t *f_done;
+  uint64_t *fc_list;
+  int *fc_n;
   int *resp_slot;
   int *resp_list;
   int64_t *ev;
diff --git a/aigar_amd/csrc/api.hip b/aigar_amd/csrc/api.hip
--- a/aigar_amd/csrc/api.hip
+++ b/aigar_amd/csrc/api.hip
@@ -551,6 +551,7 @@
   AL(occ, unsigned long long, A * d.occ_words); AL(occ_cnt, int, A * d.H);
   AL(dead, int, NP); AL(work, int, A * d.Wcap); AL(work2, int, A * d.Wcap);
   AL(f_list, int, C * FCAP); AL(f_cnt, uint8_t, C); AL(f_done, uint8_t, C);
+  AL(fc_list, uint64_t, C); AL(fc_n, int, 16);
   AL(resp_slot, int, NP); AL(resp_list, int, NP);
   AL(ev, int64_t, A * d.EVcap * 5);
   AL(o_lastfov, double, NP); AL(o_self_lf, double, NP * GG); AL(o_self_slf, double, NP * GG);
diff --git a/aigar_amd/csrc/tick.hip b/aigar_amd/csrc/tick.hip
--- a/aigar_amd/csrc/tick.hip
+++ b/aigar_amd/csrc/tick.hip
@@ -155,6 +155,25 @@
         __hip_atomic_store(&tk[8], 0, __ATOMIC_RELAXED, __HIP_MEMORY_SCOPE_AGENT);
         __builtin_amdgcn_fence(__ATOMIC_ACQUIRE, "agent");
         asm volatile("s_waitcnt vmcnt(0)" ::: "memory");
+        last = 1;
+      }
+    }
+    s_last = last;
+  }
+  __syncthreads();
+  return s_last;
+}
+__device__ inline bool last_block_sharded_relaxed(int *tk, int nblocks) {
+  __shared__ int s_last;
+  asm volatile("s_waitcnt vmcnt(0)" ::: "memory");
+  __syncthreads();
+  if (threadIdx.x == 0) {
+    const int sh = blockIdx.x & 7, members = (nblocks - sh + 7) / 8, shards = min(8, nblocks);
+    int last = 0;
+    if (__hip_atomic_fetch_add(&tk[sh], 1, __ATOMIC_RELAXED, __HIP_MEMORY_SCOPE_AGENT) == members - 1) {
+      __hip_atomic_store(&tk[sh], 0, __ATOMIC_RELAXED, __HIP_MEMORY_SCOPE_AGENT);
+      if (__hip_atomic_fetch_add(&tk[8], 1, __ATOMIC_RELAXED, __HIP_MEMORY_SCOPE_AGENT) == shards - 1) {
+        __hip_atomic_store(&tk[8], 0, __ATOMIC_RELAXED, __HIP_MEMORY_SCOPE_AGENT);
         last = 1;
       }
     }
@@ -1266,16 +1285,14 @@
 __device__ __forceinline__ int *cgrid_counts(const Dev &d, int a, int row) {
   return d.cgcnt + ((size_t)a * 2 + row) * CG_STRIDE;
 }
-__device__ __forceinline__ void cgrid_count_cell(const Dev &d, int a, size_t ci, double x, double y) {
-  const int per = kMaxCells * d.B, slot = (int)(ci / d.NP), p = (int)(ci - (size_t)slot * d.NP) - a * d.B;
+__device__ __forceinline__ int *cgrid_rank_of(const Dev &d, int a, int gp, int k) {
+  return d.c_rank + (size_t)a * kMaxCells * d.B + (size_t)k * d.B + (gp - a * d.B);
+}
+__device__ __forceinline__ void cgrid_count_cell(const Dev &d, int a, int gp, int k, double x, double y) {
   const int b = cgrid_bucket(d, x, y);
-  d.c_rank[(size_t)a * per + (size_t)slot * d.B + p] = (b << 17) | atomicAdd(&cgrid_counts(d, a, 0)[b], 1);
-}
-struct NoMid {
-  __device__ void operator()() const {}
-};
-template <class Mid = NoMid>
-__device__ void count_scan_256(int *cnt, int n, int *start, int *lds, uint16_t *bits, Mid mid = Mid()) {
+  *cgrid_rank_of(d, a, gp, k) = (b << 17) | atomicAdd(&cgrid_counts(d, a, 0)[b], 1);
+}
+__device__ void count_scan_256(int *cnt, int n, int *start, int *lds, uint16_t *bits) {
   __shared__ int wsum[4];
   const int tid = threadIdx.x, lane = tid & 63, w = tid >> 6;
   const int4 *c4 = reinterpret_cast<const int4 *>(cnt);
@@ -1286,7 +1303,6 @@
     const int j = tid * 16 + 4 * k;
     q4[k] = j < n ? c4[j >> 2] : make_int4(0, 0, 0, 0);
   }
-  mid();
 #pragma unroll
   for (int k = 0; k < 4; k++) {
     const int j = tid * 16 + 4 * k;
@@ -1311,13 +1327,7 @@
     if (lane >= off) inc += t;
   }
   if (lane == 63) wsum[w] = inc;
-  if constexpr (std::is_same<Mid, NoMid>::value) {
-    __syncthreads();
-  } else {
-    __builtin_amdgcn_fence(__ATOMIC_RELEASE, "workgroup", "local");
-    __builtin_amdgcn_s_barrier();
-    __builtin_amdgcn_fence(__ATOMIC_ACQUIRE, "workgroup", "local");
-  }
+  __syncthreads();
   int run = inc - sum;
   for (int k = 0; k < w; k++) run += wsum[k];
   const int total = wsum[0] + wsum[1] + wsum[2] + wsum[3];
@@ -1336,20 +1346,62 @@
     if (lds) lds[n] = total;
   }
 }
-template <class Mid = NoMid>
-__device__ __forceinline__ void cgrid_scan_block(const Dev &d, int a, Mid mid = Mid()) {
+__device__ __forceinline__ int cgrid_scan_per(const Dev &d) {
   const int cc = cgrid_cols(d);
-  count_scan_256(cgrid_counts(d, a, 0), cc * cc, d.cstart + (size_t)a * (d.H + 1), nullptr, nullptr, mid);
-}
-__device__ __forceinline__ void cgrid_place_player(const Dev &d, int gp, int n) {
-  const int NP = d.NP, a = gp / d.B, p = gp - a * d.B, per = kMaxCells * d.B;
-  const int *start = d.cstart + (size_t)a * (d.H + 1);
-  int *items = d.citems + (size_t)a * per;
-  for (int k = 0; k < n; k++) {
-    const int slot = d.p_list[k * NP + gp];
-    const int br = d.c_rank[(size_t)a * per + (size_t)slot * d.B + p];
-    items[start[br >> 17] + (br & 0x1FFFF)] = slot * NP + gp;
-  }
+  return (((cc * cc + 63) >> 6) + 3) & ~3;
+}
+struct CgridCounts {
+  unsigned long long q[SG_CAP / 128];
+};
+__device__ __forceinline__ void cgrid_counts_load(const Dev &d, int a, CgridCounts &c) {
+  static_assert(63 * (SG_CAP / 128) + SG_CAP / 128 <= CG_STRIDE / 2, "the loads stay inside the row");
+  const int per = cgrid_scan_per(d), lane = threadIdx.x & 63;
+  const unsigned long long *c8 =
+      reinterpret_cast<const unsigned long long *>(cgrid_counts(d, a, 0)) + (size_t)lane * (per >> 1);
+#pragma unroll
+  for (int k = 0; k < SG_CAP / 128; k++) c.q[k] = __hip_atomic_load(c8 + k, __ATOMIC_RELAXED, __HIP_MEMORY_SCOPE_AGENT);
+}
+typedef unsigned long long CgridPlane[SG_CAP / 128][64];
+__device__ __forceinline__ void cgrid_counts_stage(const Dev &d, int a, CgridPlane &pl) {
+  CgridCounts cg;
+  cgrid_counts_load(d, a, cg);
+#pragma unroll
+  for (int k = 0; k < SG_CAP / 128; k++) pl[k][threadIdx.x & 63] = cg.q[k];
+}
+__device__ __forceinline__ void cgrid_scan_wave(const Dev &d, int a, const CgridPlane &pl) {
+  const int cc = cgrid_cols(d), n = cc * cc, per = cgrid_scan_per(d), lane = threadIdx.x & 63;
+  int sum = 0;
+#pragma unroll 4
+  for (int k = 0; k < per >> 1; k++) {
+    const unsigned long long v = pl[k][lane];
+    sum += (int)(uint32_t)v + (int)(v >> 32);
+  }
+  int inc = sum;
+#pragma unroll
+  for (int off = 1; off < 64; off <<= 1) {
+    const int t = __shfl_up(inc, off);
+    if (lane >= off) inc += t;
+  }
+  int run = inc - sum;
+  int *cnt = cgrid_counts(d, a, 0), *start = d.cstart + (size_t)a * (d.H + 1);
+  const bool al = ((uintptr_t)start & 15) == 0;
+#pragma unroll 2
+  for (int k = 0; k < per >> 2; k++) {
+    const int j = lane * per + 4 * k;
+    const unsigned long long qa = pl[2 * k][lane], qb = pl[2 * k + 1][lane];
+    const int s0 = run, s1 = s0 + (int)(uint32_t)qa, s2 = s1 + (int)(qa >> 32), s3 = s2 + (int)(uint32_t)qb;
+    run = s3 + (int)(qb >> 32);
+    if (j < n) *reinterpret_cast<int4 *>(cnt + j) = make_int4(0, 0, 0, 0);
+    if (al && j + 3 <= n) {
+      *reinterpret_cast<int4 *>(start + j) = make_int4(s0, s1, s2, s3);
+    } else {
+      if (j <= n) start[j] = s0;
+      if (j + 1 <= n) start[j + 1] = s1;
+      if (j + 2 <= n) start[j + 2] = s2;
+      if (j + 3 <= n) start[j + 3] = s3;
+    }
+  }
+  if (lane == 63) start[n] = run;
 }
 
 
@@ -1505,7 +1557,7 @@
   double rmax = 0;
   for (int k = 0; k < n; k++) {
     const size_t ci = (size_t)(k < kTailRegs ? l4[k] : d.p_list[k * NP + gp]) * NP + gp;
-    cgrid_count_cell(d, a, ci, d.c_x[ci], d.c_y[ci]);
+    cgrid_count_cell(d, a, gp, k, d.c_x[ci], d.c_y[ci]);
     rmax = fmax(rmax, d.c_r[ci]);
   }
   return rmax;
@@ -1657,7 +1709,9 @@
 
 __global__ void __launch_bounds__(256) k_merge_vb(Dev d, int64_t *scr_k, int *scr_v, int fold) {
   FLOOR(2);
-  __shared__ int g_cnt[SG_CAP + 1];
+  __shared__ alignas(16) int g_cnt[SG_CAP + 1];
+  __shared__ CgridPlane s_cg[3];
+  static_assert(sizeof(g_cnt) >= sizeof(CgridPlane), "wave 0's plane");
   const int nbP = (d.NP + 255) / 256;
   if ((int)blockIdx.x >= nbP) {
     blob_grid_place(d, blockIdx.x - nbP, g_cnt);
@@ -1670,8 +1724,13 @@
     }
     wave_atomic_max_pos(&d.ctl[min(gi, d.NP - 1) / d.B].rmax_cell, rg);
   }
-  if (fold && last_block(d.ticket + 0, gridDim.x))
-    for (int a = threadIdx.x >> 6; a < d.A; a += blockDim.x >> 6) vb_serial_body(d, a, scr_k, scr_v);
+  if (last_block(d.ticket + 0, gridDim.x, fold != 0))
+    for (int a = threadIdx.x >> 6; a < d.A; a += blockDim.x >> 6) {
+      if (fold) vb_serial_body(d, a, scr_k, scr_v);
+      CgridPlane &pl = threadIdx.x < 64 ? *reinterpret_cast<CgridPlane *>(g_cnt) : s_cg[(threadIdx.x >> 6) - 1];
+      cgrid_counts_stage(d, a, pl);
+      cgrid_scan_wave(d, a, pl);
+    }
 }
 
 template <class Pred>
@@ -1770,15 +1829,15 @@
   if (count) {
 #pragma unroll
     for (int k = 0; k < kTailRegs; k++)
-      if (k < n) cgrid_count_cell(d, a, (size_t)l4[k] * NP + gp, x4[k], y4[k]);
+      if (k < n) cgrid_count_cell(d, a, gp, k, x4[k], y4[k]);
     for (int k = kTailRegs; k < n; k++) {
       const size_t ci = (size_t)d.p_list[k * NP + gp] * NP + gp;
-      cgrid_count_cell(d, a, ci, d.c_x[ci], d.c_y[ci]);
+      cgrid_count_cell(d, a, gp, k, d.c_x[ci], d.c_y[ci]);
     }
   }
   return rmax;
 }
-__device__ void pv_redo(const Dev &d, int a) {
+__device__ inline void pv_redo(const Dev &d, int a) {
   const int lane = threadIdx.x & 63;
   asm volatile("s_waitcnt vmcnt(0)" ::: "memory");
   __builtin_amdgcn_fence(__ATOMIC_ACQUIRE, "agent");
@@ -1788,10 +1847,12 @@
   asm volatile("s_waitcnt vmcnt(0)" ::: "memory");
   __builtin_amdgcn_fence(__ATOMIC_ACQUIRE, "agent");
 }
-__device__ void pv_serial_body(const Dev &d, int a, int64_t *scr_k, int *scr_v);
+__device__ inline bool pv_serial_body(const Dev &d, int a, int64_t *scr_k, int *scr_v);
 __global__ void __launch_bounds__(256) k_merge_pv(Dev d, int64_t *scr_k, int *scr_v) {
   FLOOR(2);
-  __shared__ int g_cnt[SG_CAP + 1];
+  __shared__ alignas(16) int g_cnt[SG_CAP + 1];
+  __shared__ CgridPlane s_cg[3];
+  static_assert(sizeof(g_cnt) >= sizeof(CgridPlane), "wave 0's plane");
   const int nbP = (d.NP + 255) / 256, nbB = (d.A * d.Ecap + 255) / 256, b = blockIdx.x;
   if (b < nbP) {
     const int gi = GTID;
@@ -1812,6 +1873,9 @@
   }
   if (last_block(d.ticket + 0, gridDim.x, false)) {
     __shared__ int s_work;
+    const int wv = threadIdx.x >> 6, nwv = blockDim.x >> 6, lane = threadIdx.x & 63;
+    CgridPlane &pl = wv == 0 ? *reinterpret_cast<CgridPlane *>(g_cnt) : s_cg[wv - 1];
+    if (wv < d.A) cgrid_counts_stage(d, wv, pl);
     if (threadIdx.x == 0) {
       int w = 0;
       for (int a = 0; a < d.A; a++) w |= agent_load(&d.ctl[a].n_pend) | agent_load(&d.ctl[a].n_pend2);
@@ -1819,16 +1883,22 @@
     }
     __syncthreads();
     agent_acquire_block(s_work != 0);
-    for (int a = threadIdx.x >> 6; a < d.A; a += blockDim.x >> 6) {
+    for (int a = wv; a < d.A; a += nwv) {
       const bool vb = vb_serial_body(d, a, scr_k, scr_v);
       if (__shfl(vb ? 1 : 0, 0)) pv_redo(d, a);
+      bool fresh = a != wv;
 #ifndef AIGAR_DIAG_NO_PV_SERIAL
-      pv_serial_body(d, a, scr_k, scr_v);
+      fresh |= pv_serial_body(d, a, scr_k, scr_v);
 #endif
-    }
-  }
-}
-__device__ void pv_serial_body(const Dev &d, int a, int64_t *scr_k, int *scr_v) {
+      if (fresh) {
+        asm volatile("s_waitcnt vmcnt(0)" ::: "memory");
+        cgrid_counts_stage(d, a, pl);
+      }
+      cgrid_scan_wave(d, a, pl);
+    }
+  }
+}
+__device__ inline bool pv_serial_body(const Dev &d, int a, int64_t *scr_k, int *scr_v) {
   const int lane = threadIdx.x & 63;
   const unsigned long long lt = (1ull << lane) - 1;
   ArenaCtl &c = d.ctl[a];
@@ -1838,7 +1908,7 @@
     c.n_pend2 = 0;
     c.stat[1] += nw;
   }
-  if (nw == 0) return;
+  if (nw == 0) return false;
   const int NP = d.NP;
   int *w = d.work2 + (size_t)a * d.Wcap;
   int64_t *ck = scr_k + (size_t)a * d.Wcap;
@@ -1940,7 +2010,7 @@
           d.c_seq[ni] = seq;
           d.c_flags[ni] = F_ALIVE | F_INHASH | F_NEW;
           d.c_active[ni] = 0;
-          if (lane == 0) cgrid_count_cell(d, a, ni, px, py);
+          if (lane == 0) cgrid_count_cell(d, a, gp, ncur + k, px, py);
           d.p_list[(ncur + k) * NP + gp] = (uint8_t)slot;
         }
         d.p_ncells[gp] = ncur + n_new;
@@ -1948,6 +2018,7 @@
     }
     for (int k = 0; k < d.p_ncells[gp]; k++) d.c_flags[(size_t)d.p_list[k * NP + gp] * NP + gp] &= ~F_NEW;
   }
+  return true;
 }
 
 constexpr int kBlobBit = 1 << 30;
@@ -2051,9 +2122,18 @@
 }
 
 constexpr int PREP_CAND = 128;
+constexpr int FS_CAP = 512;
+struct FoodSerialLds {
+  int64_t *key;
+  int *val, *srt;
+  double *x, *y, *m, *r;
+};
 constexpr int PREP_WAVES = 1;
 __device__ __forceinline__ double tile_rall() { return sqrt(kMaxMass / kPi) * (1 + 1e-9); }
-__global__ void __launch_bounds__(256, 4) k_food_prep(Dev d, int rounds, int resume) {
+__device__ __forceinline__ void food_commit_block(const Dev &d, int rounds, int64_t *scr_k, int *scr_v,
+                                                  const FoodSerialLds &L PT_PARAMS);
+__global__ void __launch_bounds__(256, 4) k_food_prep(Dev d, int rounds, int resume, int commit, int64_t *scr_k,
+                                                      int *scr_v) {
   FLOOR(4);
   TILE_GATE(d);
   __shared__ int64_t s_seq[4][PREP_CAND];
@@ -2061,39 +2141,47 @@
   __shared__ int s_idx[4][PREP_CAND];
   __shared__ uint8_t s_sel[4][PREP_CAND];
   __shared__ uint64_t s_bm[4][64];
-  const bool head = !resume && (int)blockIdx.x < d.A;
+  __shared__ double s_fr[FS_CAP];
+  static_assert(4 * PREP_CAND == FS_CAP && sizeof(s_bm) == FS_CAP * sizeof(int), "food_serial_body's arrays alias these");
   PT_BEGIN(0);
   const int w = threadIdx.x >> 6, lane = threadIdx.x & 63;
+  auto prep_wave = [&]() {
   const int wi = xcd_block(blockIdx.x, gridDim.x) * 4 + w, gp = wi / PREP_WAVES,
             h = wi - gp * PREP_WAVES;
   static_assert(PREP_WAVES == 1, "prep_multi assumes one wave per player");
-  if (gp < d.NP && gp % d.B == 0 && h == 0 && lane == 0) d.ctl[gp / d.B].food_undone[1] = 0;
-  if (gp >= d.NP && !head) return;
-  const int gpl = min(gp, d.NP - 1);
-  const int NP = d.NP, a = gpl / d.B;
-  const int v_first = d.p_list[h * NP + gpl];
-  const int v_slot = d.p_list[(lane < kMaxCells ? lane : 0) * NP + gpl];
+  if (!commit && gp < d.NP && gp % d.B == 0 && h == 0 && lane == 0) d.ctl[gp / d.B].food_undone[1] = 0;
+  if (gp >= d.NP) return;
+  const int NP = d.NP, a = gp / d.B;
+  const int v_first = d.p_list[h * NP + gp];
+  const int v_slot = d.p_list[(lane < kMaxCells ? lane : 0) * NP + gp];
+  const int pl_br = *cgrid_rank_of(d, a, gp, lane < kMaxCells ? lane : 0);
   s_bm[w][lane] = d.bmap[(size_t)a * 64 + lane];
-  const bool alive = d.p_alive[gpl];
+  const bool alive = d.p_alive[gp];
   Food F(d, a);
   const uint32_t base = d.ctl[a].food_round;
-  const int v_n = d.p_ncells[gpl];
-  if (head) {
-    double t0 = 0, t1 = 0, t2 = 0, t3 = 0;
-    long long t4 = 0;
-    cgrid_scan_block(d, blockIdx.x, [&] {
-      if (gp < NP && alive && v_n > 0) {
-        const size_t ci = (size_t)v_first * NP + gp;
-        t0 = d.c_x[ci];
-        t1 = d.c_y[ci];
-        t2 = d.c_m[ci];
-        t3 = d.c_r[ci];
-        t4 = d.c_seq[ci];
-      }
-    });
-    asm volatile("" ::"v"(t0), "v"(t1), "v"(t2), "v"(t3), "v"(t4));
-    if (gp >= NP) return;
-  }
+  const int v_n = d.p_ncells[gp];
+  const bool plc = !resume && alive && lane < v_n;
+  int pl_st = 0;
+  if (plc) pl_st = d.cstart[(size_t)a * (d.H + 1) + (pl_br >> 17)];
+  bool placed = false;
+  auto place_store = [&]() {
+    if (placed) return;
+    placed = true;
+    if (plc) d.citems[(size_t)a * kMaxCells * d.B + pl_st + (pl_br & 0x1FFFF)] = v_slot * NP + gp;
+  };
+  auto st_done = [&](size_t ci, uint8_t v) {
+    if (commit) __hip_atomic_store(&d.f_done[ci], v, __ATOMIC_RELAXED, __HIP_MEMORY_SCOPE_AGENT);
+    else d.f_done[ci] = v;
+  };
+  auto st_int = [&](int *p, int v) {
+    if (commit) __hip_atomic_store(p, v, __ATOMIC_RELAXED, __HIP_MEMORY_SCOPE_AGENT);
+    else *p = v;
+  };
+  auto list_cell = [&](size_t kc, int slot, int cnt) {
+    const int e = atomicAdd(&d.fc_n[0], 1);
+    __hip_atomic_store(&d.fc_list[e], (uint64_t)kc | (uint64_t)slot << 32 | (uint64_t)cnt << 40, __ATOMIC_RELAXED,
+                       __HIP_MEMORY_SCOPE_AGENT);
+  };
   const int s_first = uni(v_first);
   const int n0 = uni(v_n);
   const int n = alive ? n0 : 0;
@@ -2209,13 +2297,15 @@
       uint64_t key = food_key(base + rounds + 1, prio);
       if (lane == 0) {
         d.f_cnt[kc] = kOverflow;
-        d.f_done[ci] = 0;
-        int wi = atomicAdd(&d.ctl[a].n_pend, 1);
+        st_done(ci, 0);
+        int ao = a;
+        asm volatile("" : "+v"(ao));
+        int wi = atomicAdd(&d.ctl[ao].n_pend, 1);
         if (wi < d.Wcap) {
-          d.work[(size_t)a * d.Wcap + wi] = (int)ci;
-          d.work2[(size_t)a * d.Wcap + wi] = (int)prio;
+          st_int(&d.work[(size_t)ao * d.Wcap + wi], (int)ci);
+          st_int(&d.work2[(size_t)ao * d.Wcap + wi], (int)prio);
         } else {
-          set_err(d, a, ERR_WORK_CAP);
+          set_err(d, ao, ERR_WORK_CAP);
         }
       }
       F.walk_pellets(q, [&](bool valid, int j) {
@@ -2236,13 +2326,18 @@
         int64_t sq = s_seq[w][i];
         int rk = 0;
         for (int jj = 0; jj < cnt; jj++) rk += (s_sel[w][jj] && s_seq[w][jj] < sq);
-        lst[rk] = s_idx[w][i];
+        st_int(&lst[rk], s_idx[w][i]);
         atomicMax((unsigned long long *)F.owner(s_idx[w][i]), (unsigned long long)key);
       }
     }
     if (lane == 0) {
       d.f_cnt[kc] = (uint8_t)nsel;
-      d.f_done[ci] = (nsel == 0);
+      if (nsel == 0) {
+        d.f_done[ci] = 1;
+      } else {
+        st_done(ci, 0);
+        if (commit) list_cell(kc, (int)(ci / NP), nsel);
+      }
     }
     wave_sync_lds();
     PT_MARK(0, 6);
@@ -2255,6 +2350,7 @@
     const size_t ci = (size_t)(has ? slot : s_first) * NP + gp;
     const double x = d.c_x[ci], y = d.c_y[ci], m = d.c_m[ci], r = d.c_r[ci];
     PT_MARK(0, 2);
+    place_store();
     const Rect q = footprint(x, y, r, d.size);
     const Span sp = grid_span(q, 1, d.cols, 0);
     const int ngrid = sp.by1 - sp.by0 + 1;
@@ -2372,14 +2468,19 @@
         int rk = 0;
         for (int jj = cps; jj < cps + cpc; jj++) rk += ((s_sel[w][jj] & 0x80) && s_seq[w][jj] < sq);
         const int j = s_idx[w][i];
-        d.f_list[((size_t)cc * NP + gp) * FCAP + rk] = j;
+        st_int(&d.f_list[((size_t)cc * NP + gp) * FCAP + rk], j);
         atomicMax((unsigned long long *)F.owner(j),
                   (unsigned long long)food_key(base + 1, (uint32_t)p * kMaxCells + cc));
       }
     }
     if (has && sub == 0) {
       d.f_cnt[(size_t)g * NP + gp] = (uint8_t)nsel;
-      d.f_done[ci] = (nsel == 0);
+      if (nsel == 0) {
+        d.f_done[ci] = 1;
+      } else {
+        st_done(ci, 0);
+        if (commit) list_cell((size_t)g * NP + gp, slot, nsel);
+      }
     }
     PT_MARK(0, 6);
     return true;
@@ -2388,7 +2489,22 @@
     if (prep_multi()) return;
     wave_sync_lds();
   }
+  if (!resume && !placed && n > 0) {
+    const size_t ci = (size_t)s_first * NP + gp;
+    const double t0 = d.c_x[ci], t1 = d.c_y[ci], t2 = d.c_m[ci], t3 = d.c_r[ci];
+    const long long t4 = d.c_seq[ci];
+    place_store();
+    asm volatile("" ::"v"(t0), "v"(t1), "v"(t2), "v"(t3), "v"(t4));
+  }
   for (int k = 0; k < n; k++) prep_cell(gp, k, (size_t)(k == 0 ? s_first : uni((int)d.p_list[k * NP + gp])) * NP + gp);
+  };
+  prep_wave();
+  if (!commit) return;
+  if (!last_block_sharded_relaxed(d.fc_n + 4, gridDim.x)) return;
+  PT_MARK(0, 7);
+  food_commit_block(d, rounds, scr_k, scr_v,
+                    FoodSerialLds{&s_seq[0][0], &s_idx[0][0], reinterpret_cast<int *>(&s_bm[0][0]), &s_x[0][0], &s_y[0][0],
+                                  &s_m[0][0], s_fr} PT_ARGS);
 }
 __device__ __forceinline__ void food_eat(const Dev &d, const Food &F, int a, int j, uint32_t prio, int t,
                                          int64_t cseq, int64_t fseq, double fm, double &m, double &r, int &eaten,
@@ -2406,14 +2522,15 @@
   F.kill(j);
   eaten += bl ? 0 : 1;
 }
-struct FoodBatch {
-  int j[kTailRegs];
-  bool al[kTailRegs];
-  double x[kTailRegs], y[kTailRegs], m[kTailRegs], r[kTailRegs];
-  int64_t sq[kTailRegs];
+template <int N>
+struct FoodBatchT {
+  int j[N];
+  bool al[N];
+  double x[N], y[N], m[N], r[N];
+  int64_t sq[N];
   __device__ void load(const Dev &d, const Food &F, const int *jv, int n) {
 #pragma unroll
-    for (int k = 0; k < kTailRegs; k++) {
+    for (int k = 0; k < N; k++) {
       j[k] = jv[k];
       al[k] = false;
       x[k] = y[k] = m[k] = r[k] = 0;
@@ -2426,12 +2543,18 @@
     }
   }
 };
+using FoodBatch = FoodBatchT<kTailRegs>;
+constexpr int kCommitRegs = 2;
+template <bool AG>
+constexpr int commit_regs() { return AG ? kCommitRegs : kTailRegs; }
 struct EaterIn {
   double x, y, m, r;
   int64_t seq;
 };
-__device__ double food_eat_loop(const Dev &d, const Food &F, int a, size_t ci, const EaterIn &cell, uint32_t prio,
-                                const int *lst, int cnt, FoodBatch &fb) {
+template <bool AG>
+__device__ __forceinline__ double food_eat_loop(const Dev &d, const Food &F, int a, size_t ci, const EaterIn &cell, uint32_t prio,
+                                const int *lst, int cnt, FoodBatchT<commit_regs<AG>()> &fb) {
+  constexpr int N = commit_regs<AG>();
   const double x = cell.x, y = cell.y;
   double m = cell.m, r = cell.r;
   const int64_t cseq = cell.seq;
@@ -2439,16 +2562,16 @@
   int eaten = 0;
   bool blobs = false, ate = false;
   Rect qb{};
-  for (int t0 = 0; t0 < cnt; t0 += kTailRegs) {
+  for (int t0 = 0; t0 < cnt; t0 += N) {
     if (t0 > 0) {
-      int jv[kTailRegs];
-#pragma unroll
-      for (int k = 0; k < kTailRegs; k++) jv[k] = t0 + k < cnt ? lst[t0 + k] : 0;
+      int jv[N];
+#pragma unroll
+      for (int k = 0; k < N; k++) jv[k] = t0 + k < cnt ? (AG ? agent_load(lst + t0 + k) : lst[t0 + k]) : 0;
       fb.load(d, F, jv, cnt - t0);
     }
-    int kp[kTailRegs], nkp = 0;
-#pragma unroll
-    for (int k = 0; k < kTailRegs; k++) {
+    int kp[N], nkp = 0;
+#pragma unroll
+    for (int k = 0; k < N; k++) {
       kp[k] = -1;
       const int t = t0 + k, j = fb.j[k];
       if (t >= cnt) continue;
@@ -2483,7 +2606,7 @@
     if (nkp) {
       int b = atomicAdd(&d.ctl[a].n_kill, nkp);
 #pragma unroll
-      for (int k = 0; k < kTailRegs; k++)
+      for (int k = 0; k < N; k++)
         if (kp[k] >= 0) {
           if (b < d.Pcap) d.kill_list[(size_t)a * d.Pcap + b] = kp[k];
           else set_err(d, a, ERR_PELLET_CAP);
@@ -2497,7 +2620,69 @@
   if (eaten) atomicAdd(&d.ctl[a].n_pel_eaten, eaten);
   return ate ? r : 0.0;
 }
-__device__ double food_commit_player(const Dev &d, int gp, int round, int last, int place PT_PARAMS) {
+template <bool AG>
+__device__ __forceinline__ int food_commit_cell(const Dev &d, const Food &F, int a, int gp, int k, int slot, int cnt,
+                                                const int *l4, int round, int last, double &rgrow PT_PARAMS) {
+  constexpr int N = commit_regs<AG>();
+  const int NP = d.NP, p = gp - a * d.B;
+  ArenaCtl &c = d.ctl[a];
+  const size_t kc = (size_t)k * NP + gp;
+  const int *lst = d.f_list + kc * FCAP;
+  const size_t ci = (size_t)slot * NP + gp;
+  uint32_t prio = (uint32_t)p * kMaxCells + k;
+  bool own = true;
+  FoodBatchT<N> fb;
+  EaterIn cell;
+  auto owner_of = [&](int j) -> uint64_t {
+    return AG ? __hip_atomic_load(F.owner(j), __ATOMIC_RELAXED, __HIP_MEMORY_SCOPE_AGENT) : *F.owner(j);
+  };
+  {
+    const bool done = AG ? false : d.f_done[ci];
+    cell.x = d.c_x[ci];
+    cell.y = d.c_y[ci];
+    cell.m = d.c_m[ci];
+    cell.r = d.c_r[ci];
+    cell.seq = d.c_seq[ci];
+    uint64_t key = food_key(c.food_round + round, prio);
+    uint64_t kw[N];
+#pragma unroll
+    for (int t = 0; t < N; t++) kw[t] = t < cnt ? owner_of(l4[t]) : key;
+    fb.load(d, F, l4, cnt);
+#pragma unroll
+    for (int t = 0; t < N; t++) own &= kw[t] == key;
+    if (done) return 0;
+    for (int t = N; t < cnt && own; t++) own = (owner_of(AG ? agent_load(lst + t) : lst[t]) == key);
+  }
+  PT_MARKW(4, 3);
+  if (own) {
+    rgrow = fmax(rgrow, food_eat_loop<AG>(d, F, a, ci, cell, prio, lst, cnt, fb));
+    d.f_done[ci] = 1;
+    PT_MARKW(4, 4);
+    return 0;
+  }
+  if (!last) {
+    uint64_t key = food_key(c.food_round + round + 1, prio);
+    for (int t = 0; t < cnt; t++)
+      atomicMax((unsigned long long *)F.owner(AG ? agent_load(lst + t) : lst[t]), (unsigned long long)key);
+    atomicAdd(&c.food_undone[round % 3], 1);
+    return 1;
+  }
+  int w = atomicAdd(&c.n_pend, 1);
+  if (w < d.Wcap) {
+    int *w1 = &d.work[(size_t)a * d.Wcap + w], *w2 = &d.work2[(size_t)a * d.Wcap + w];
+    if (AG) {
+      __hip_atomic_store(w1, (int)ci, __ATOMIC_RELAXED, __HIP_MEMORY_SCOPE_AGENT);
+      __hip_atomic_store(w2, (int)prio, __ATOMIC_RELAXED, __HIP_MEMORY_SCOPE_AGENT);
+    } else {
+      *w1 = (int)ci;
+      *w2 = (int)prio;
+    }
+  } else {
+    set_err(d, a, ERR_WORK_CAP);
+  }
+  return 2;
+}
+__device__ double food_commit_player(const Dev &d, int gp, int round, int last PT_PARAMS) {
   const int NP = d.NP, a = gp / d.B, p = gp - a * d.B;
   ArenaCtl &c = d.ctl[a];
   const bool alive = d.p_alive[gp];
@@ -2507,7 +2692,6 @@
   int l4_first[kTailRegs];
 #pragma unroll
   for (int t = 0; t < kTailRegs; t++) l4_first[t] = d.f_list[(size_t)gp * FCAP + t];
-  if (place && alive) cgrid_place_player(d, gp, n);
   if (round > 1 && c.food_undone[(round - 1) % 3] == 0) return 0;
   if (p == 0) c.food_undone[(round + 1) % 3] = 0;
   if (!alive) return 0;
@@ -2527,59 +2711,26 @@
     }
     PT_MARKW(4, 2);
     if (cnt == 0 || cnt == kOverflow) continue;
-    const size_t ci = (size_t)slot * NP + gp;
-    uint32_t prio = (uint32_t)p * kMaxCells + k;
-    bool own = true;
-    FoodBatch fb;
-    EaterIn cell;
-    bool done;
-    {
-      done = d.f_done[ci];
-      cell.x = d.c_x[ci];
-      cell.y = d.c_y[ci];
-      cell.m = d.c_m[ci];
-      cell.r = d.c_r[ci];
-      cell.seq = d.c_seq[ci];
-      uint64_t key = food_key(d.ctl[a].food_round + round, prio);
-      uint64_t kw[kTailRegs];
-#pragma unroll
-      for (int t = 0; t < kTailRegs; t++) kw[t] = t < cnt ? *F.owner(l4[t]) : key;
-      fb.load(d, F, l4, cnt);
-#pragma unroll
-      for (int t = 0; t < kTailRegs; t++) own &= kw[t] == key;
-      if (done) continue;
-      for (int t = kTailRegs; t < cnt && own; t++) own = (*F.owner(lst[t]) == key);
-    }
-    PT_MARKW(4, 3);
-    if (own) {
-      rgrow = fmax(rgrow, food_eat_loop(d, F, a, ci, cell, prio, lst, cnt, fb));
-      d.f_done[ci] = 1;
-      PT_MARKW(4, 4);
-    } else if (!last) {
-      uint64_t key = food_key(d.ctl[a].food_round + round + 1, prio);
-      for (int t = 0; t < cnt; t++) atomicMax((unsigned long long *)F.owner(lst[t]), (unsigned long long)key);
-      atomicAdd(&c.food_undone[round % 3], 1);
-    } else {
-      int w = atomicAdd(&d.ctl[a].n_pend, 1);
-      if (w < d.Wcap) {
-        d.work[(size_t)a * d.Wcap + w] = (int)ci;
-        d.work2[(size_t)a * d.Wcap + w] = (int)prio;
-      } else {
-        set_err(d, a, ERR_WORK_CAP);
-      }
-    }
+    food_commit_cell<false>(d, F, a, gp, k, slot, cnt, l4, round, last, rgrow PT_ARGS);
   }
   return rgrow;
 }
-__device__ void food_serial_body(const Dev &d, int a, int64_t *scr_k, int *scr_v, int rounds);
+__device__ __forceinline__ void food_serial_body(const Dev &d, int a, int64_t *scr_k, int *scr_v, int rounds,
+                                                 const FoodSerialLds &L);
+__device__ void food_serial_own(const Dev &d, int a, int64_t *scr_k, int *scr_v, int rounds) {
+  __shared__ int64_t s_key[FS_CAP];
+  __shared__ int s_val[FS_CAP], s_srt[FS_CAP];
+  __shared__ double s_x[FS_CAP], s_y[FS_CAP], s_m[FS_CAP], s_r[FS_CAP];
+  food_serial_body(d, a, scr_k, scr_v, rounds, FoodSerialLds{s_key, s_val, s_srt, s_x, s_y, s_m, s_r});
+}
 __global__ void __launch_bounds__(256) k_food_commit(Dev d, int round, int last, int64_t *scr_k, int *scr_v,
-                                                     int rounds, int fold, int place) {
+                                                     int rounds, int fold) {
   FLOOR(5);
   TILE_GATE(d);
   const int ncommit = (d.NP + 255) / 256;
   PT_BEGIN(4);
   const int gp = GTID;
-  const double rg = gp < d.NP ? food_commit_player(d, gp, round, last, place PT_ARGS) : 0.0;
+  const double rg = gp < d.NP ? food_commit_player(d, gp, round, last PT_ARGS) : 0.0;
   PT_MARK(4, round < 7 ? round : 7);
   wave_atomic_max_pos(&d.ctl[min(gp, d.NP - 1) / d.B].rmax_cell, rg);
   PT_MARK(4, 5);
@@ -2593,15 +2744,55 @@
     __syncthreads();
     agent_acquire_block(s_work != 0);
     if (threadIdx.x < 64)
-      for (int a = 0; a < d.A; a++) food_serial_body(d, a, scr_k, scr_v, rounds);
+      for (int a = 0; a < d.A; a++) food_serial_own(d, a, scr_k, scr_v, rounds);
     PT_MARK(4, 6);
   }
 }
-constexpr int FS_CAP = 512;
-__device__ void food_serial_body(const Dev &d, int a, int64_t *scr_k, int *scr_v, int rounds) {
-  __shared__ int64_t s_key[FS_CAP];
-  __shared__ int s_val[FS_CAP], s_srt[FS_CAP];
-  __shared__ double s_x[FS_CAP], s_y[FS_CAP], s_m[FS_CAP], s_r[FS_CAP];
+__device__ __forceinline__ void food_commit_block(const Dev &d, int rounds, int64_t *scr_k, int *scr_v,
+                                                  const FoodSerialLds &L PT_PARAMS) {
+  const int tid = threadIdx.x;
+  const int N = agent_load(&d.fc_n[0]);
+  for (int a = tid; a < d.A; a += blockDim.x)
+    __hip_atomic_store(&d.ctl[a].food_undone[1], 0, __ATOMIC_RELAXED, __HIP_MEMORY_SCOPE_AGENT);
+  asm volatile("s_waitcnt vmcnt(0)" ::: "memory");
+  __syncthreads();
+  for (int round = 1; round <= rounds; round++) {
+    for (int a = tid; a < d.A; a += blockDim.x)
+      if (round == 1 || agent_load(&d.ctl[a].food_undone[(round - 1) % 3]) != 0)
+        __hip_atomic_store(&d.ctl[a].food_undone[(round + 1) % 3], 0, __ATOMIC_RELAXED, __HIP_MEMORY_SCOPE_AGENT);
+    int undone = 0;
+    for (int i = tid; i < N; i += blockDim.x) {
+      const uint64_t e = __hip_atomic_load(&d.fc_list[i], __ATOMIC_RELAXED, __HIP_MEMORY_SCOPE_AGENT);
+      if (e == 0) continue;
+      const size_t kc = (size_t)(e & 0xFFFFFFFFull);
+      const int slot = (int)(e >> 32) & 0xFF, cnt = (int)(e >> 40);
+      const int k = (int)(kc / d.NP), gp = (int)(kc - (size_t)k * d.NP), a = gp / d.B;
+      int l4[kCommitRegs];
+#pragma unroll
+      for (int t = 0; t < kCommitRegs; t++) l4[t] = agent_load(d.f_list + kc * FCAP + t);
+      PT_MARKW(4, 2);
+      const Food F(d, a);
+      double rgrow = 0;
+      const int st = food_commit_cell<true>(d, F, a, gp, k, slot, cnt, l4, round, round == rounds, rgrow PT_ARGS);
+      if (rgrow > 0) atomic_max_pos(&d.ctl[a].rmax_cell, rgrow);
+      if (st == 1) undone = 1;
+      else __hip_atomic_store(&d.fc_list[i], (uint64_t)0, __ATOMIC_RELAXED, __HIP_MEMORY_SCOPE_AGENT);
+    }
+    PT_MARK(4, round < 3 ? round : 3);
+    asm volatile("s_waitcnt vmcnt(0)" ::: "memory");
+    if (!__syncthreads_or(undone)) break;
+  }
+  PT_MARK(4, 5);
+  if (tid == 0) __hip_atomic_store(&d.fc_n[0], 0, __ATOMIC_RELAXED, __HIP_MEMORY_SCOPE_AGENT);
+  if (tid < 64)
+    for (int a = 0; a < d.A; a++) food_serial_body(d, a, scr_k, scr_v, rounds, L);
+  PT_MARK(4, 6);
+}
+__device__ __forceinline__ void food_serial_body(const Dev &d, int a, int64_t *scr_k, int *scr_v, int rounds,
+                                                 const FoodSerialLds &L) {
+  int64_t *const s_key = L.key;
+  int *const s_val = L.val, *const s_srt = L.srt;
+  double *const s_x = L.x, *const s_y = L.y, *const s_m = L.m, *const s_r = L.r;
   const int lane = threadIdx.x & 63;
   ArenaCtl &c = d.ctl[a];
   const int nw = min(agent_load(&c.n_pend), d.Wcap);
@@ -2618,8 +2809,8 @@
   int *wp = d.work2 + (size_t)a * d.Wcap;
   if (nw <= FS_CAP) {
     for (int k = lane; k < nw; k += 64) {
-      s_val[k] = w[k];
-      s_key[k] = wp[k];
+      s_val[k] = agent_load(w + k);
+      s_key[k] = agent_load(wp + k);
     }
     wave_fence();
     for (int k = lane; k < nw; k += 64) {
@@ -2635,7 +2826,10 @@
     }
   } else if (lane == 0) {
     int64_t *ck = scr_k + (size_t)a * d.Wcap;
-    for (int k = 0; k < nw; k++) ck[k] = wp[k];
+    for (int k = 0; k < nw; k++) {
+      ck[k] = agent_load(wp + k);
+      w[k] = agent_load(w + k);
+    }
     isort_kv(ck, w, nw);
     for (int k = 0; k < nw; k++) wp[k] = (int)ck[k];
   }
@@ -2747,7 +2941,7 @@
 }
 __global__ void __launch_bounds__(64) k_food_serial(Dev d, int64_t *scr_k, int *scr_v, int rounds) {
   TILE_GATE(d);
-  food_serial_body(d, blockIdx.x, scr_k, scr_v, rounds);
+  food_serial_own(d, blockIdx.x, scr_k, scr_v, rounds);
 }
 
 __device__ __forceinline__ Rect cell_rect(const Dev &d, size_t ci) { return footprint(d.c_x[ci], d.c_y[ci], d.c_r[ci], d.size); }
@@ -4662,11 +4856,13 @@
 static void launch_food(const Dev &d, hipStream_t s, int rounds, Scratch scr, int resume = 0, int fold = 0) {
   rounds = std::max(rounds, 1);
   const int g = nblk(d.NP, 256);
-  hipLaunchKernelGGL(k_food_prep, dim3(std::max(nblk((long)d.NP * PREP_WAVES, 4), resume ? 0 : d.A)), dim3(256), 0, s, d,
-                     rounds, resume);
+  const int commit = !d.tiled && !resume && fold;
+  hipLaunchKernelGGL(k_food_prep, dim3(nblk((long)d.NP * PREP_WAVES, 4)), dim3(256), 0, s, d, rounds, resume, commit,
+                     scr.k, scr.v);
+  if (commit) return;
   for (int r = 1; r <= rounds; r++) {
     hipLaunchKernelGGL(k_food_commit, dim3(g), dim3(256), 0, s, d, r, r == rounds ? 1 : 0, scr.k, scr.v, rounds,
-                       fold && r == rounds ? 1 : 0, r == 1 && !resume ? 1 : 0);
+                       fold && r == rounds ? 1 : 0);
   }
   if (!fold) hipLaunchKernelGGL(k_food_serial, dim3(d.A), dim3(64), 0, s, d, scr.k, scr.v, rounds);
 }
```
